# nv-nguyen/gigapose

Hardware: NVIDIA H100
Metric: detections/sec (224x224 crops, 162-template bank) (higher is better)
Workload: dtype f32 (a1, a4, a6: bf16 hi/lo split x3 on tensor cores with fp32 accumulate = fp32-faithful; a5, a7-a9: fp32)

## Files before the change

gigapose_b200/csrc/api.cu:

```cuda
#include "../../include/gigapose_b200.h"
#include "gigapose_kernels.h"

#include <atomic>
#include <dlfcn.h>
#include <cstdarg>
#include <cstdio>
#include <cstdlib>
#include <cstring>
#include <new>
#include <string>

int gp_internal_make_map_nhwc(CUtensorMap* map, void* ptr, uint64_t C, uint64_t W, uint64_t H, uint64_t N, uint32_t out_w,
                              uint32_t out_h, uint32_t stride);
int gp_internal_make_map_raw(CUtensorMap* map, void* ptr, int rank, const uint64_t* dims, const uint64_t* strides_bytes,
                             const uint32_t* box, const uint32_t* elem_strides);
int gp_internal_make_map_ex(CUtensorMap* map, void* ptr, uint64_t rows, uint64_t cols, uint32_t box_cols, uint32_t box_rows,
                            int swizzle_bytes);
int gp_internal_make_map(CUtensorMap* map, void* ptr, uint64_t rows, uint64_t cols, uint32_t box_rows);

namespace {

thread_local std::string g_last_error;
std::atomic<uint64_t> g_launches{0};

int fail(int code, const char* fmt, ...) {
  char buf[512];
  va_list ap;
  va_start(ap, fmt);
  vsnprintf(buf, sizeof(buf), fmt, ap);
  va_end(ap);
  g_last_error = buf;
  return code;
}

#define GP_CUDA(expr)                                                                                     \
  do {                                                                                                    \
    cudaError_t _e = (expr);                                                                              \
    if (_e != cudaSuccess) return fail(GP_ERR_CUDA, "%s failed: %s", #expr, cudaGetErrorString(_e));     \
  } while (0)

constexpr size_t kAlign = 1024;
inline size_t align_up(size_t x) { return (x + kAlign - 1) / kAlign * kAlign; }

struct Carver {
  uint8_t* base;
  size_t off = 0;
  explicit Carver(void* b) : base(static_cast<uint8_t*>(b)) {}
  template <typename T>
  T* take(size_t count) {
    T* p = base ? reinterpret_cast<T*>(base + off) : nullptr;
    off += align_up(count * sizeof(T));
    return p;
  }
};

typedef CUresult (*EncodeTiledFn)(CUtensorMap*, CUtensorMapDataType, cuuint32_t, void*, const cuuint64_t*,
                                  const cuuint64_t*, const cuuint32_t*, const cuuint32_t*, CUtensorMapInterleave,
                                  CUtensorMapSwizzle, CUtensorMapL2promotion, CUtensorMapFloatOOBfill);

EncodeTiledFn get_encode_fn() {
  static EncodeTiledFn fn = nullptr;
  if (!fn) {
    void* p = nullptr;
    cudaDriverEntryPointQueryResult q;
    if (cudaGetDriverEntryPoint("cuTensorMapEncodeTiled", &p, cudaEnableDefault, &q) == cudaSuccess &&
        q == cudaDriverEntryPointSuccess)
      fn = reinterpret_cast<EncodeTiledFn>(p);
  }
  return fn;
}

}

int gp_internal_fail(int code, const char* fmt, ...) {
  char buf[512];
  va_list ap;
  va_start(ap, fmt);
  vsnprintf(buf, sizeof(buf), fmt, ap);
  va_end(ap);
  g_last_error = buf;
  return code;
}
void gp_internal_count_launches(int n) { g_launches += n; }
namespace gp {
bool pdl_enabled() {
  const char* ev = getenv("GIGAPOSE_PDL");
  return ev ? (ev[0] != '0') : false;
}
}

int gp_internal_make_map_ex(CUtensorMap* map, void* ptr, uint64_t rows, uint64_t cols, uint32_t box_cols, uint32_t box_rows,
                            int swizzle_bytes) {
  EncodeTiledFn enc = get_encode_fn();
  if (!enc) return fail(GP_ERR_UNSUPPORTED, "cuTensorMapEncodeTiled not available from this driver");
  cuuint64_t dims[2] = {cols, rows};
  cuuint64_t strides[1] = {cols * sizeof(uint16_t)};
  cuuint32_t box[2] = {box_cols, box_rows};
  cuuint32_t estr[2] = {1, 1};
  const CUtensorMapSwizzle sw = swizzle_bytes == 128 ? CU_TENSOR_MAP_SWIZZLE_128B : CU_TENSOR_MAP_SWIZZLE_64B;
  CUresult r = enc(map, CU_TENSOR_MAP_DATA_TYPE_BFLOAT16, 2, ptr, dims, strides, box, estr, CU_TENSOR_MAP_INTERLEAVE_NONE, sw,
                   CU_TENSOR_MAP_L2_PROMOTION_L2_128B, CU_TENSOR_MAP_FLOAT_OOB_FILL_NONE);
  if (r != CUDA_SUCCESS) return fail(GP_ERR_CUDA, "cuTensorMapEncodeTiled failed with CUresult %d", (int)r);
  return GP_OK;
}
int gp_internal_make_map_nhwc(CUtensorMap* map, void* ptr, uint64_t C, uint64_t W, uint64_t H, uint64_t N, uint32_t out_w,
                              uint32_t out_h, uint32_t stride) {
  EncodeTiledFn enc = get_encode_fn();
  if (!enc) return fail(GP_ERR_UNSUPPORTED, "cuTensorMapEncodeTiled not available from this driver");
  cuuint64_t dims[4] = {C, W, H, N};
  cuuint64_t strides[3] = {C * sizeof(uint16_t), W * C * sizeof(uint16_t), H * W * C * sizeof(uint16_t)};
  cuuint32_t box[4] = {32, out_w * stride, out_h * stride, 1};
  cuuint32_t estr[4] = {1, stride, stride, 1};
  CUresult r = enc(map, CU_TENSOR_MAP_DATA_TYPE_BFLOAT16, 4, ptr, dims, strides, box, estr, CU_TENSOR_MAP_INTERLEAVE_NONE,
                   CU_TENSOR_MAP_SWIZZLE_64B, CU_TENSOR_MAP_L2_PROMOTION_L2_128B, CU_TENSOR_MAP_FLOAT_OOB_FILL_NONE);
  if (r != CUDA_SUCCESS) return fail(GP_ERR_CUDA, "cuTensorMapEncodeTiled (NHWC) failed with CUresult %d", (int)r);
  return GP_OK;
}
int gp_internal_make_map_raw(CUtensorMap* map, void* ptr, int rank, const uint64_t* dims, const uint64_t* strides_bytes,
                             const uint32_t* box, const uint32_t* elem_strides) {
  EncodeTiledFn enc = get_encode_fn();
  if (!enc) return fail(GP_ERR_UNSUPPORTED, "cuTensorMapEncodeTiled not available from this driver");
  cuuint64_t d[5], st[4];
  cuuint32_t b[5], es[5];
  for (int i = 0; i < rank; ++i) { d[i] = dims[i]; b[i] = box[i]; es[i] = elem_strides[i]; if (i + 1 < rank) st[i] = strides_bytes[i]; }
  CUresult r = enc(map, CU_TENSOR_MAP_DATA_TYPE_BFLOAT16, rank, ptr, d, st, b, es, CU_TENSOR_MAP_INTERLEAVE_NONE,
                   CU_TENSOR_MAP_SWIZZLE_64B, CU_TENSOR_MAP_L2_PROMOTION_L2_128B, CU_TENSOR_MAP_FLOAT_OOB_FILL_NONE);
  if (r != CUDA_SUCCESS) return fail(GP_ERR_CUDA, "cuTensorMapEncodeTiled (raw, rank %d) failed with CUresult %d", rank, (int)r);
  return GP_OK;
}
int gp_internal_make_map(CUtensorMap* map, void* ptr, uint64_t rows, uint64_t cols, uint32_t box_rows) {
  return gp_internal_make_map_ex(map, ptr, rows, cols, 32, box_rows, 64);
}

namespace {

int make_plane_map(CUtensorMap* map, void* ptr, uint64_t images, uint32_t box_rows) {
  return gp_internal_make_map_ex(map, ptr, images * 32ull * GP_NUM_PATCHES, 32, 32, box_rows, 64);
}

struct Bank {
  uint16_t *hi, *lo;
  float* mask16;
  float* ist;
  float *K, *M, *pose;
};

struct Workspace {
  uint16_t *q_hi, *q_lo;
  float* q_mask16;
  float* q_ist;
  int *perm, *q_obj;
  float* sim_avg;
  float* rec_score;
  uint8_t *rec_idx, *rec_valid;
  float* c_score; int* c_id; float* c_pts_score; uint8_t *c_idx, *c_valid;
  int* row_count; int* row_ids; float *hidden1, *hidden2;
  uint16_t *mlp_a_hi, *mlp_a_lo;
  uint16_t *w1_hi, *w1_lo, *w2s_hi, *w2s_lo, *w2i_hi, *w2i_lo;
  float* bias1;
};

void carve_bank(Carver& c, const gp_config_t& cfg, Bank* b) {
  const size_t OT = (size_t)cfg.num_objects * cfg.num_templates;
  const size_t OTg = (size_t)cfg.num_objects * cfg.num_templates_global;
  Bank tmp;
  tmp.hi = c.take<uint16_t>(OT * GP_NUM_PATCHES * GP_AE_DIM);
  tmp.lo = c.take<uint16_t>(OT * GP_NUM_PATCHES * GP_AE_DIM);
  tmp.mask16 = c.take<float>(OT * GP_NUM_PATCHES);
  tmp.ist = c.take<float>((cfg.ist_bank_global ? OTg : OT) * GP_NUM_PATCHES * GP_IST_DIM);
  tmp.K = c.take<float>((size_t)cfg.num_objects * 9);
  tmp.M = c.take<float>(OTg * 9);
  tmp.pose = c.take<float>(OTg * 16);
  if (b) *b = tmp;
}

void carve_workspace(Carver& c, const gp_config_t& cfg, Workspace* w) {
  const size_t Bm = cfg.max_batch, T = cfg.num_templates, k = cfg.top_k;
  Workspace tmp;
  tmp.q_hi = c.take<uint16_t>(Bm * GP_NUM_PATCHES * GP_AE_DIM);
  tmp.q_lo = c.take<uint16_t>(Bm * GP_NUM_PATCHES * GP_AE_DIM);
  tmp.q_mask16 = c.take<float>(Bm * GP_NUM_PATCHES);
  tmp.q_ist = c.take<float>(Bm * GP_NUM_PATCHES * GP_IST_DIM);
  tmp.perm = c.take<int>(Bm);
  tmp.q_obj = c.take<int>(Bm);
  tmp.sim_avg = c.take<float>(Bm * T);
  tmp.rec_score = c.take<float>(Bm * T * GP_NUM_PATCHES);
  tmp.rec_idx = c.take<uint8_t>(Bm * T * GP_NUM_PATCHES);
  tmp.rec_valid = c.take<uint8_t>(Bm * T * GP_NUM_PATCHES);
  tmp.c_score = c.take<float>(Bm * k);
  tmp.c_id = c.take<int>(Bm * k);
  tmp.c_pts_score = c.take<float>(Bm * k * GP_NUM_PATCHES);
  tmp.c_idx = c.take<uint8_t>(Bm * k * GP_NUM_PATCHES);
  tmp.c_valid = c.take<uint8_t>(Bm * k * GP_NUM_PATCHES);
  tmp.row_count = c.take<int>(1);
  tmp.row_ids = c.take<int>(Bm * k * GP_NUM_PATCHES);
  tmp.hidden1 = c.take<float>(Bm * k * GP_NUM_PATCHES * 1024);
  tmp.hidden2 = c.take<float>(Bm * k * GP_NUM_PATCHES * 512);
  tmp.mlp_a_hi = c.take<uint16_t>(Bm * k * GP_NUM_PATCHES * 512);
  tmp.mlp_a_lo = c.take<uint16_t>(Bm * k * GP_NUM_PATCHES * 512);
  tmp.w1_hi = c.take<uint16_t>(1024 * 512);
  tmp.w1_lo = c.take<uint16_t>(1024 * 512);
  tmp.w2s_hi = c.take<uint16_t>(256 * 512);
  tmp.w2s_lo = c.take<uint16_t>(256 * 512);
  tmp.w2i_hi = c.take<uint16_t>(256 * 512);
  tmp.w2i_lo = c.take<uint16_t>(256 * 512);
  tmp.bias1 = c.take<float>(1024);
  if (w) *w = tmp;
}

int validate(const gp_config_t* cfg) {
  if (!cfg) return fail(GP_ERR_INVALID, "null config");
  if (cfg->abi_version != GP_ABI_VERSION) return fail(GP_ERR_INVALID, "ABI version mismatch: %d vs %d", cfg->abi_version, GP_ABI_VERSION);
  if (cfg->num_objects < 1 || cfg->num_templates < 1 || cfg->max_batch < 1)
    return fail(GP_ERR_INVALID, "num_objects, num_templates and max_batch must be >= 1");
  if (cfg->top_k < 1 || cfg->top_k > 32) return fail(GP_ERR_INVALID, "top_k must be in [1,32]");
  if (cfg->num_templates_global < cfg->num_templates) return fail(GP_ERR_INVALID, "num_templates_global < num_templates");
  if (cfg->num_templates_global < cfg->top_k) return fail(GP_ERR_INVALID, "fewer templates than top_k (torch.topk would raise)");
  if (cfg->template_id_stride < 1 || cfg->template_id_offset < 0) return fail(GP_ERR_INVALID, "bad template id stride/offset");
  if (cfg->patch_size < 1) return fail(GP_ERR_INVALID, "patch_size must be >= 1");
  if (cfg->sim_threshold != cfg->sim_threshold) return fail(GP_ERR_INVALID, "sim_threshold is NaN");
  if (cfg->precision != GP_PRECISION_FP32_SPLIT && cfg->precision != GP_PRECISION_BF16)
    return fail(GP_ERR_INVALID, "unknown precision %d", cfg->precision);
  if (cfg->ist_bank_global != 0 && cfg->ist_bank_global != 1) return fail(GP_ERR_INVALID, "ist_bank_global must be 0 or 1");
  if ((size_t)cfg->num_objects * cfg->num_templates * GP_NUM_PATCHES * 32 >= (1ull << 31))
    return fail(GP_ERR_INVALID, "bank has too many rows for 32-bit TMA coordinates");
  return GP_OK;
}

}

struct gp_context {
  gp_config_t cfg;
  int num_sms;
  Bank bank;
  Workspace ws;
  CUtensorMap tm_q_hi, tm_q_lo, tm_t_hi, tm_t_lo;
  int mlp_tc;
  CUtensorMap tm_ma_hi, tm_ma_lo;
  CUtensorMap tm_h1s_hi, tm_h1s_lo, tm_h1i_hi, tm_h1i_lo;
  CUtensorMap tm_w1_hi, tm_w1_lo, tm_w2s_hi, tm_w2s_lo, tm_w2i_hi, tm_w2i_lo;
  gp::IstMlpWeights mlp;
  bool mlp_set;
  int cur_B;
  void* nccl_comm;
  int rank, world;
};

namespace {
typedef int (*NcclAllGatherFn)(const void*, void*, size_t, int, void*, cudaStream_t);
typedef const char* (*NcclErrFn)(int);
NcclAllGatherFn g_allgather = nullptr;
NcclErrFn g_nccl_err = nullptr;
int resolve_nccl() {
  if (g_allgather) return GP_OK;
  void* sym = dlsym(RTLD_DEFAULT, "ncclAllGather");
  void* lib = nullptr;
  if (!sym) {
    lib = dlopen("libnccl.so.2", RTLD_NOW | RTLD_GLOBAL);
    if (lib) sym = dlsym(lib, "ncclAllGather");
  }
  if (!sym) return fail(GP_ERR_UNSUPPORTED, "ncclAllGather not found: load libnccl.so.2 (e.g. import torch) before gp_comm_init");
  g_allgather = reinterpret_cast<NcclAllGatherFn>(sym);
  void* es = dlsym(RTLD_DEFAULT, "ncclGetErrorString");
  if (!es && lib) es = dlsym(lib, "ncclGetErrorString");
  g_nccl_err = reinterpret_cast<NcclErrFn>(es);
  return GP_OK;
}
}

extern "C" {

const char* gp_last_error(void) { return g_last_error.c_str(); }
int gp_abi_version(void) { return GP_ABI_VERSION; }
uint64_t gp_launch_count(void) { return g_launches.load(); }

int gp_query_sizes(const gp_config_t* cfg, size_t* bank_bytes, size_t* workspace_bytes) {
  if (int e = validate(cfg)) return e;
  Carver cb(nullptr), cw(nullptr);
  carve_bank(cb, *cfg, nullptr);
  carve_workspace(cw, *cfg, nullptr);
  if (bank_bytes) *bank_bytes = cb.off;
  if (workspace_bytes) *workspace_bytes = cw.off;
  return GP_OK;
}

int gp_create(const gp_config_t* cfg, void* bank_mem, void* workspace_mem, gp_handle_t* out) {
  if (int e = validate(cfg)) return e;
  if (!bank_mem || !workspace_mem || !out) return fail(GP_ERR_INVALID, "null pointer argument");
  if (((uintptr_t)bank_mem | (uintptr_t)workspace_mem) & (kAlign - 1))
    return fail(GP_ERR_INVALID, "bank and workspace must be %zu-byte aligned", kAlign);
  GP_CUDA(cudaSetDevice(cfg->device));
  cudaDeviceProp prop;
  GP_CUDA(cudaGetDeviceProperties(&prop, cfg->device));
  if (prop.major != 9 || prop.minor != 0)
    return fail(GP_ERR_UNSUPPORTED, "device %d is sm_%d%d; this library contains sm_90a code only", cfg->device,
                prop.major, prop.minor);
  if ((int)prop.sharedMemPerBlockOptin < gp::sim_search_smem_bytes())
    return fail(GP_ERR_UNSUPPORTED, "device offers %zu B of shared memory per block, kernel needs %d",
                prop.sharedMemPerBlockOptin, gp::sim_search_smem_bytes());
  gp_context* h = new (std::nothrow) gp_context();
  if (!h) return fail(GP_ERR_INVALID, "out of host memory");
  h->cfg = *cfg;
  h->num_sms = prop.multiProcessorCount;
  h->mlp_set = false;
  h->cur_B = 0;
  {
    const char* ev = getenv("GIGAPOSE_MLP_SIMT");
    h->mlp_tc = ev ? (ev[0] == '0') : 0;
  }
  h->nccl_comm = nullptr;
  h->rank = 0;
  h->world = 1;
  Carver cb(bank_mem), cw(workspace_mem);
  carve_bank(cb, *cfg, &h->bank);
  carve_workspace(cw, *cfg, &h->ws);
  const uint64_t bank_rows = (uint64_t)cfg->num_objects * cfg->num_templates;
  const uint64_t q_rows = (uint64_t)cfg->max_batch;
  int e;
  if ((e = make_plane_map(&h->tm_t_hi, h->bank.hi, bank_rows, 256)) || (e = make_plane_map(&h->tm_t_lo, h->bank.lo, bank_rows, 256)) ||
      (e = make_plane_map(&h->tm_q_hi, h->ws.q_hi, q_rows, 128)) || (e = make_plane_map(&h->tm_q_lo, h->ws.q_lo, q_rows, 128))) {
    delete h;
    return e;
  }
  {
    const uint64_t rows = (uint64_t)cfg->max_batch * cfg->top_k * GP_NUM_PATCHES;
    uint16_t* h1_hi = reinterpret_cast<uint16_t*>(h->ws.hidden1);
    uint16_t* h1_lo = h1_hi + rows * 1024;
    const uint64_t dims[2] = {512, rows}, strides[1] = {1024 * sizeof(uint16_t)};
    const uint32_t box[2] = {32, 128}, estr[2] = {1, 1};
    int e;
    if ((e = gp_internal_make_map(&h->tm_ma_hi, h->ws.mlp_a_hi, rows, 512, 128)) || (e = gp_internal_make_map(&h->tm_ma_lo, h->ws.mlp_a_lo, rows, 512, 128)) ||
        (e = gp_internal_make_map_raw(&h->tm_h1s_hi, h1_hi, 2, dims, strides, box, estr)) ||
        (e = gp_internal_make_map_raw(&h->tm_h1s_lo, h1_lo, 2, dims, strides, box, estr)) ||
        (e = gp_internal_make_map_raw(&h->tm_h1i_hi, h1_hi + 512, 2, dims, strides, box, estr)) ||
        (e = gp_internal_make_map_raw(&h->tm_h1i_lo, h1_lo + 512, 2, dims, strides, box, estr)) ||
        (e = gp_internal_make_map(&h->tm_w1_hi, h->ws.w1_hi, 1024, 512, 256)) || (e = gp_internal_make_map(&h->tm_w1_lo, h->ws.w1_lo, 1024, 512, 256)) ||
        (e = gp_internal_make_map(&h->tm_w2s_hi, h->ws.w2s_hi, 256, 512, 256)) || (e = gp_internal_make_map(&h->tm_w2s_lo, h->ws.w2s_lo, 256, 512, 256)) ||
        (e = gp_internal_make_map(&h->tm_w2i_hi, h->ws.w2i_hi, 256, 512, 256)) || (e = gp_internal_make_map(&h->tm_w2i_lo, h->ws.w2i_lo, 256, 512, 256))) {
      delete h;
      return e;
    }
  }
  *out = h;
  return GP_OK;
}

int gp_destroy(gp_handle_t h) {
  delete h;
  return GP_OK;
}

namespace {
int split_features(const float* feat, int feat_layout, long long n_imgs, int norm_passes, uint16_t* hi, uint16_t* lo, cudaStream_t s) {
  const long long rows = n_imgs * GP_NUM_PATCHES;
  cudaError_t e;
  if (feat_layout == GP_LAYOUT_CHANNEL_MAJOR)
    e = gp::launch_split_descriptors(feat, rows, GP_AE_DIM, GP_NUM_PATCHES, (long long)GP_NUM_PATCHES * GP_AE_DIM, 1, GP_NUM_PATCHES,
                                     norm_passes, 1, hi, lo, nullptr, s);
  else if (feat_layout == GP_LAYOUT_PATCH_MAJOR)
    e = gp::launch_split_descriptors(feat, rows, GP_AE_DIM, GP_NUM_PATCHES, (long long)GP_NUM_PATCHES * GP_AE_DIM, GP_AE_DIM, 1,
                                     norm_passes, 1, hi, lo, nullptr, s);
  else if (feat_layout == GP_LAYOUT_VIT_TOKENS)
    e = gp::launch_split_descriptors(feat + GP_AE_DIM, rows, GP_AE_DIM, GP_NUM_PATCHES, (long long)(GP_NUM_PATCHES + 1) * GP_AE_DIM,
                                     GP_AE_DIM, 1, norm_passes, 1, hi, lo, nullptr, s);
  else
    return fail(GP_ERR_INVALID, "unknown feature layout %d", feat_layout);
  if (e != cudaSuccess) return fail(GP_ERR_CUDA, "descriptor split failed: %s", cudaGetErrorString(e));
  return GP_OK;
}
}

int gp_normalize_patch_tokens(int b, const float* x_prenorm, float* out, void* stream) {
  if (!x_prenorm || !out || b < 1) return fail(GP_ERR_INVALID, "bad argument");
  GP_CUDA(gp::launch_split_descriptors(x_prenorm + GP_AE_DIM, (long long)b * GP_NUM_PATCHES, GP_AE_DIM, GP_NUM_PATCHES,
                                       (long long)(GP_NUM_PATCHES + 1) * GP_AE_DIM, GP_AE_DIM, 1, 1, 0, nullptr, nullptr, out,
                                       static_cast<cudaStream_t>(stream)));
  g_launches += 1;
  return GP_OK;
}

int gp_bank_write(gp_handle_t h, int obj, int tmpl0, int n, const float* feat, int feat_layout, int norm_passes,
                  const float* mask, int H, int W, const float* ist_feat, void* stream) {
  if (!h) return fail(GP_ERR_INVALID, "null handle");
  const gp_config_t& c = h->cfg;
  if (obj < 0 || obj >= c.num_objects || tmpl0 < 0 || n < 1 || tmpl0 + n > c.num_templates)
    return fail(GP_ERR_INVALID, "template range [%d,%d) of object %d outside the bank (%d x %d)", tmpl0, tmpl0 + n, obj,
                c.num_objects, c.num_templates);
  if (!feat || !mask) return fail(GP_ERR_INVALID, "feat and mask are required");
  if (H < 16 || W < 16) return fail(GP_ERR_INVALID, "mask must be at least 16x16");
  if (norm_passes < 0 || norm_passes > 2) return fail(GP_ERR_INVALID, "norm_passes must be 0, 1 or 2");
  cudaStream_t s = static_cast<cudaStream_t>(stream);
  const size_t slot = (size_t)obj * c.num_templates + tmpl0;
  const size_t plane_off = slot * GP_NUM_PATCHES * GP_AE_DIM;
  if (int e = split_features(feat, feat_layout, n, norm_passes, h->bank.hi + plane_off, h->bank.lo + plane_off, s)) return e;
  GP_CUDA(gp::launch_sample_mask16(mask, n, H, W, h->bank.mask16 + slot * GP_NUM_PATCHES, s));
  g_launches += 2;
  if (ist_feat) {
    if (c.ist_bank_global) return fail(GP_ERR_INVALID, "cfg.ist_bank_global = 1: write IST features with gp_bank_write_ist (global ids)");
    GP_CUDA(gp::launch_transpose_cp(ist_feat, n, GP_IST_DIM, h->bank.ist + slot * GP_NUM_PATCHES * GP_IST_DIM, s));
    g_launches += 1;
  }
  return GP_OK;
}

int gp_bank_write_ist(gp_handle_t h, int obj, int tmpl0, int n, const float* ist_feat, int ist_layout, void* stream) {
  if (!h || !ist_feat) return fail(GP_ERR_INVALID, "null argument");
  const gp_config_t& c = h->cfg;
  const int Ti = c.ist_bank_global ? c.num_templates_global : c.num_templates;
  if (obj < 0 || obj >= c.num_objects || tmpl0 < 0 || n < 1 || tmpl0 + n > Ti)
    return fail(GP_ERR_INVALID, "IST template range [%d,%d) of object %d outside the bank (%d x %d)", tmpl0, tmpl0 + n, obj,
                c.num_objects, Ti);
  cudaStream_t s = static_cast<cudaStream_t>(stream);
  float* dst = h->bank.ist + ((size_t)obj * Ti + tmpl0) * GP_NUM_PATCHES * GP_IST_DIM;
  if (ist_layout == GP_LAYOUT_CHANNEL_MAJOR) {
    GP_CUDA(gp::launch_transpose_cp(ist_feat, n, GP_IST_DIM, dst, s));
    g_launches += 1;
  } else if (ist_layout == GP_LAYOUT_PATCH_MAJOR) {
    GP_CUDA(cudaMemcpyAsync(dst, ist_feat, (size_t)n * GP_NUM_PATCHES * GP_IST_DIM * sizeof(float), cudaMemcpyDeviceToDevice, s));
  } else {
    return fail(GP_ERR_INVALID, "unknown IST feature layout %d", ist_layout);
  }
  return GP_OK;
}

int gp_bank_set_poses(gp_handle_t h, const float* K, const float* M, const float* poses, void* stream) {
  if (!h || !K || !M || !poses) return fail(GP_ERR_INVALID, "null argument");
  const gp_config_t& c = h->cfg;
  cudaStream_t s = static_cast<cudaStream_t>(stream);
  const size_t OTg = (size_t)c.num_objects * c.num_templates_global;
  GP_CUDA(cudaMemcpyAsync(h->bank.K, K, (size_t)c.num_objects * 9 * sizeof(float), cudaMemcpyDeviceToDevice, s));
  GP_CUDA(cudaMemcpyAsync(h->bank.M, M, OTg * 9 * sizeof(float), cudaMemcpyDeviceToDevice, s));
  GP_CUDA(cudaMemcpyAsync(h->bank.pose, poses, OTg * 16 * sizeof(float), cudaMemcpyDeviceToDevice, s));
  return GP_OK;
}

static constexpr float kMlpWeightScale = 64.0f;

int gp_set_ist_weights(gp_handle_t h, const float* const w[12], int use_tanh, void* stream) {
  if (!h || !w) return fail(GP_ERR_INVALID, "null argument");
  for (int i = 0; i < 12; ++i)
    if (!w[i]) return fail(GP_ERR_INVALID, "IST weight pointer %d is null", i);
  gp::IstMlpWeights& m = h->mlp;
  m.s_w1 = w[0]; m.s_b1 = w[1]; m.s_w2 = w[2]; m.s_b2 = w[3]; m.s_w3 = w[4]; m.s_b3 = w[5];
  m.i_w1 = w[6]; m.i_b1 = w[7]; m.i_w2 = w[8]; m.i_b2 = w[9]; m.i_w3 = w[10]; m.i_b3 = w[11];
  m.use_tanh = use_tanh;
  cudaStream_t s = static_cast<cudaStream_t>(stream);
  Workspace& ws = h->ws;
  GP_CUDA(gp::launch_split_planes(w[0], 512, 512, 512, ws.w1_hi, ws.w1_lo, s, true, kMlpWeightScale));
  GP_CUDA(gp::launch_split_planes(w[6], 512, 512, 512, ws.w1_hi + 512 * 512, ws.w1_lo + 512 * 512, s, true, kMlpWeightScale));
  GP_CUDA(gp::launch_split_planes(w[2], 256, 512, 512, ws.w2s_hi, ws.w2s_lo, s, true, kMlpWeightScale));
  GP_CUDA(gp::launch_split_planes(w[8], 256, 512, 512, ws.w2i_hi, ws.w2i_lo, s, true, kMlpWeightScale));
  GP_CUDA(cudaMemcpyAsync(ws.bias1, w[1], 512 * sizeof(float), cudaMemcpyDeviceToDevice, s));
  GP_CUDA(cudaMemcpyAsync(ws.bias1 + 512, w[7], 512 * sizeof(float), cudaMemcpyDeviceToDevice, s));
  g_launches += 4;
  h->mlp_set = true;
  return GP_OK;
}

int gp_set_queries(gp_handle_t h, int B, const float* q_feat, int feat_layout, int norm_passes, const float* q_mask,
                   int H, int W, const int32_t* q_obj, void* stream) {
  if (!h || !q_feat || !q_mask || !q_obj) return fail(GP_ERR_INVALID, "null argument");
  if (B < 1 || B > h->cfg.max_batch) return fail(GP_ERR_INVALID, "batch %d outside [1, max_batch=%d]", B, h->cfg.max_batch);
  if (H < 16 || W < 16) return fail(GP_ERR_INVALID, "mask must be at least 16x16");
  if (norm_passes < 0 || norm_passes > 2) return fail(GP_ERR_INVALID, "norm_passes must be 0, 1 or 2");
  cudaStream_t s = static_cast<cudaStream_t>(stream);
  if (int e = split_features(q_feat, feat_layout, B, norm_passes, h->ws.q_hi, h->ws.q_lo, s)) return e;
  GP_CUDA(gp::launch_sample_mask16(q_mask, B, H, W, h->ws.q_mask16, s));
  GP_CUDA(gp::launch_object_order(q_obj, B, h->cfg.num_objects, h->ws.q_obj, h->ws.perm, s));
  g_launches += 3;
  h->cur_B = B;
  return GP_OK;
}

static int run_sim(gp_context* h, int B, cudaStream_t s, float* debug_tile = nullptr) {
  gp::SimSearchParams p;
  p.num_items = B * h->cfg.num_templates;
  p.B = B;
  p.T = h->cfg.num_templates;
  p.perm = h->ws.perm;
  p.q_obj = h->ws.q_obj;
  p.q_mask = h->ws.q_mask16;
  p.bank_mask = h->bank.mask16;
  p.sim_threshold = h->cfg.sim_threshold;
  p.patch_threshold = h->cfg.patch_threshold;
  p.passes = h->cfg.precision == GP_PRECISION_FP32_SPLIT ? 3 : 1;
  p.sim_avg = h->ws.sim_avg;
  p.rec_score = h->ws.rec_score;
  p.rec_idx = h->ws.rec_idx;
  p.rec_valid = h->ws.rec_valid;
  p.debug_tile = debug_tile;
  GP_CUDA(gp::launch_sim_search(h->tm_q_hi, h->tm_q_lo, h->tm_t_hi, h->tm_t_lo, p, h->num_sms, s));
  g_launches += 1;
  return GP_OK;
}

int gp_sim_candidates(gp_handle_t h, int B, const gp_candidates_t* out, void* stream) {
  if (!h || !out) return fail(GP_ERR_INVALID, "null argument");
  if (B != h->cur_B) return fail(GP_ERR_STATE, "gp_set_queries staged %d queries, search asked for %d", h->cur_B, B);
  cudaStream_t s = static_cast<cudaStream_t>(stream);
  if (int e = run_sim(h, B, s)) return e;
  gp::TopkSelectParams t;
  t.B = B; t.T = h->cfg.num_templates; t.k = h->cfg.top_k;
  t.id_stride = h->cfg.template_id_stride; t.id_offset = h->cfg.template_id_offset;
  t.sim_avg = h->ws.sim_avg; t.rec_score = h->ws.rec_score; t.rec_idx = h->ws.rec_idx; t.rec_valid = h->ws.rec_valid;
  t.cand_score = out->score; t.cand_id = out->id; t.cand_pts_score = out->pts_score; t.cand_idx = out->idx;
  t.cand_valid = out->valid;
  GP_CUDA(gp::launch_topk_select(t, s));
  g_launches += 1;
  return GP_OK;
}

int gp_topk_merge(gp_handle_t h, int B, int G, const gp_candidates_t* g, size_t rank_stride_bytes,
                  const gp_matches_t* out, float* out_rel_scale, float* out_rel_inplane, void* stream) {
  if (!h || !g || !out) return fail(GP_ERR_INVALID, "null argument");
  if (B < 1 || G < 1 || G * h->cfg.top_k > 64) return fail(GP_ERR_INVALID, "B=%d G=%d: need G*k <= 64", B, G);
  gp::TopkMergeParams m;
  m.B = B; m.k = h->cfg.top_k; m.G = G; m.rank_stride_bytes = rank_stride_bytes;
  m.cand_score = g->score; m.cand_id = g->id; m.cand_pts_score = g->pts_score; m.cand_idx = g->idx; m.cand_valid = g->valid;
  m.cand_rel_scale = g->rel_scale; m.cand_rel_inplane = g->rel_inplane;
  m.out_rel_scale = out_rel_scale; m.out_rel_inplane = out_rel_inplane;
  m.id_src = reinterpret_cast<long long*>(out->id_src); m.score_src = out->score_src; m.score_pts = out->score_pts;
  m.tar_pts = reinterpret_cast<long long*>(out->tar_pts); m.src_pts = reinterpret_cast<long long*>(out->src_pts);
  GP_CUDA(gp::launch_topk_merge_expand(m, static_cast<cudaStream_t>(stream)));
  g_launches += 1;
  return GP_OK;
}

int gp_sim_topk(gp_handle_t h, int B, const gp_matches_t* out, void* stream) {
  if (!h || !out) return fail(GP_ERR_INVALID, "null argument");
  gp_candidates_t c;
  c.score = h->ws.c_score; c.id = h->ws.c_id; c.pts_score = h->ws.c_pts_score; c.idx = h->ws.c_idx; c.valid = h->ws.c_valid;
  c.rel_scale = nullptr; c.rel_inplane = nullptr;
  if (int e = gp_sim_candidates(h, B, &c, stream)) return e;
  return gp_topk_merge(h, B, 1, &c, 0, out, nullptr, nullptr, stream);
}

int gp_ist_mlp(gp_handle_t h, int b0, int n, const float* q_ist, int ist_layout, const gp_matches_t* m, float* rel_scale,
               float* rel_inplane, void* stream) {
  if (!h || !q_ist || !m || !rel_scale || !rel_inplane) return fail(GP_ERR_INVALID, "null argument");
  if (!h->mlp_set) return fail(GP_ERR_STATE, "gp_set_ist_weights has not been called");
  if (b0 < 0 || n < 1 || b0 + n > h->cur_B)
    return fail(GP_ERR_STATE, "gp_set_queries staged %d queries, gp_ist_mlp asked for [%d,%d)", h->cur_B, b0, b0 + n);
  cudaStream_t s = static_cast<cudaStream_t>(stream);
  const float* q_pm = q_ist;
  if (ist_layout == GP_LAYOUT_CHANNEL_MAJOR) {
    GP_CUDA(gp::launch_transpose_cp(q_ist, n, GP_IST_DIM, h->ws.q_ist, s));
    q_pm = h->ws.q_ist;
    g_launches += 1;
  } else if (ist_layout != GP_LAYOUT_PATCH_MAJOR) {
    return fail(GP_ERR_INVALID, "unknown IST feature layout %d", ist_layout);
  }
  const gp_config_t& c = h->cfg;
  gp::IstMlpParams p;
  p.B = n; p.k = c.top_k;
  if (c.ist_bank_global) { p.T = c.num_templates_global; p.id_stride = 1; p.id_offset = 0; }
  else { p.T = c.num_templates; p.id_stride = c.template_id_stride; p.id_offset = c.template_id_offset; }
  p.id_src = reinterpret_cast<const long long*>(m->id_src);
  p.src_pts = reinterpret_cast<const long long*>(m->src_pts);
  p.tar_pts = reinterpret_cast<const long long*>(m->tar_pts);
  p.q_obj = h->ws.q_obj + b0; p.q_ist = q_pm; p.bank_ist = h->bank.ist;
  p.rel_scale = rel_scale; p.rel_inplane = rel_inplane;
  p.row_count = h->ws.row_count; p.row_ids = h->ws.row_ids; p.hidden1 = h->ws.hidden1; p.hidden2 = h->ws.hidden2;
  if (!h->mlp_tc) {
    GP_CUDA(gp::launch_ist_mlp(h->mlp, p, s));
    g_launches += 4;
    return GP_OK;
  }
  const int rows = n * c.top_k * GP_NUM_PATCHES;
  const uint64_t max_rows = (uint64_t)c.max_batch * c.top_k * GP_NUM_PATCHES;
  uint16_t* h1_hi = reinterpret_cast<uint16_t*>(h->ws.hidden1);
  uint16_t* h1_lo = h1_hi + max_rows * 1024;
  float* h2s = h->ws.hidden2;
  float* h2i = h->ws.hidden2 + max_rows * 256;
  GP_CUDA(gp::launch_mlp_gather_planes(p, h->ws.mlp_a_hi, h->ws.mlp_a_lo, s));
  gp::GemmParams g{};
  g.passes = 3; g.f16 = 1; g.acc_scale = 1.0f / kMlpWeightScale; g.m_dev = h->ws.row_count;
  g.M = rows; g.N = 1024; g.K = 512; g.mode = gp::GEMM_PLANES_RELU; g.bias = h->ws.bias1; g.out_hi = h1_hi; g.out_lo = h1_lo;
  GP_CUDA(gp::launch_vit_gemm(h->tm_ma_hi, h->tm_ma_lo, h->tm_w1_hi, h->tm_w1_lo, g, h->num_sms, s));
  g = gp::GemmParams{};
  g.passes = 3; g.f16 = 1; g.acc_scale = 1.0f / kMlpWeightScale; g.m_dev = h->ws.row_count;
  g.M = rows; g.N = 256; g.K = 512; g.mode = gp::GEMM_ROWS_F32_RELU; g.bias = h->mlp.s_b2; g.x = h2s;
  GP_CUDA(gp::launch_vit_gemm(h->tm_h1s_hi, h->tm_h1s_lo, h->tm_w2s_hi, h->tm_w2s_lo, g, h->num_sms, s));
  g.bias = h->mlp.i_b2; g.x = h2i;
  GP_CUDA(gp::launch_vit_gemm(h->tm_h1i_hi, h->tm_h1i_lo, h->tm_w2i_hi, h->tm_w2i_lo, g, h->num_sms, s));
  GP_CUDA(gp::launch_mlp_head_rows(h->mlp, p, h2s, h2i, s));
  g_launches += 6;
  return GP_OK;
}

int gp_ransac(int n, float pixel_threshold, int patch_size, const int64_t* src_pts, const int64_t* tar_pts,
              const float* rel_scale, const float* rel_inplane, const gp_ransac_out_t* out, void* stream) {
  if (!src_pts || !tar_pts || !rel_scale || !rel_inplane || !out || !out->inlier_count || !out->M || !out->failed ||
      !out->inlier_src_pts || !out->inlier_tar_pts || !out->inlier_scores)
    return fail(GP_ERR_INVALID, "null argument");
  if (n < 1) return fail(GP_ERR_INVALID, "n must be >= 1");
  gp::RansacParams p;
  p.n = n; p.pixel_threshold = pixel_threshold; p.patch_size = patch_size;
  p.src_pts = reinterpret_cast<const long long*>(src_pts);
  p.tar_pts = reinterpret_cast<const long long*>(tar_pts);
  p.rel_scale = rel_scale; p.rel_inplane = rel_inplane;
  p.M = out->M; p.failed = out->failed;
  p.in_src = reinterpret_cast<long long*>(out->inlier_src_pts);
  p.in_tar = reinterpret_cast<long long*>(out->inlier_tar_pts);
  p.in_score = reinterpret_cast<long long*>(out->inlier_scores);
  p.in_count = out->inlier_count;
  GP_CUDA(gp::launch_ransac(p, static_cast<cudaStream_t>(stream)));
  g_launches += 1;
  return GP_OK;
}

int gp_pose_recover(int B, int k, int num_templates, const int32_t* q_obj, const float* q_K, const float* q_M,
                    const int64_t* id_src, const float* M, const float* tmpl_K, const float* tmpl_M,
                    const float* tmpl_pose, float* poses, void* stream) {
  if (!q_obj || !q_K || !q_M || !id_src || !M || !tmpl_K || !tmpl_M || !tmpl_pose || !poses)
    return fail(GP_ERR_INVALID, "null argument");
  if (B < 1 || k < 1 || num_templates < 1) return fail(GP_ERR_INVALID, "B, k and num_templates must be >= 1");
  GP_CUDA(gp::launch_pose_only(B * k, k, num_templates, q_obj, q_K, q_M, reinterpret_cast<const long long*>(id_src), M,
                               tmpl_K, tmpl_M, tmpl_pose, poses, static_cast<cudaStream_t>(stream)));
  g_launches += 1;
  return GP_OK;
}

int gp_sort_and_pose(gp_handle_t h, int b0, int n, int sort_by_inliers, const float* q_K, const float* q_M,
                     const gp_matches_t* m, const float* rel_scale, const float* rel_inplane, const gp_ransac_out_t* r,
                     const gp_predictions_t* o, void* stream) {
  if (!h || !q_K || !q_M || !m || !rel_scale || !rel_inplane || !r || !o) return fail(GP_ERR_INVALID, "null argument");
  if (b0 < 0 || n < 1 || b0 + n > h->cur_B)
    return fail(GP_ERR_STATE, "gp_set_queries staged %d queries, gp_sort_and_pose asked for [%d,%d)", h->cur_B, b0, b0 + n);
  gp::PoseParams p;
  p.B = n; p.k = h->cfg.top_k; p.T = h->cfg.num_templates_global;
  p.sort = sort_by_inliers ? 1 : 0;
  p.q_obj = h->ws.q_obj + b0; p.q_K = q_K; p.q_M = q_M;
  p.tmpl_K = h->bank.K; p.tmpl_M = h->bank.M; p.tmpl_pose = h->bank.pose;
  p.in_count = r->inlier_count;
  p.id_src = reinterpret_cast<const long long*>(m->id_src); p.score_src = m->score_src; p.score_pts = m->score_pts;
  p.tar_pts = reinterpret_cast<const long long*>(m->tar_pts); p.src_pts = reinterpret_cast<const long long*>(m->src_pts);
  p.rel_scale = rel_scale; p.rel_inplane = rel_inplane;
  p.M = r->M; p.failed = r->failed;
  p.in_src = reinterpret_cast<const long long*>(r->inlier_src_pts);
  p.in_tar = reinterpret_cast<const long long*>(r->inlier_tar_pts);
  p.in_score = reinterpret_cast<const long long*>(r->inlier_scores);
  p.o_id_src = reinterpret_cast<long long*>(o->matches.id_src); p.o_score_src = o->matches.score_src;
  p.o_score_pts = o->matches.score_pts;
  p.o_tar_pts = reinterpret_cast<long long*>(o->matches.tar_pts); p.o_src_pts = reinterpret_cast<long long*>(o->matches.src_pts);
  p.o_rel_scale = o->rel_scale; p.o_rel_inplane = o->rel_inplane;
  p.o_M = o->ransac.M; p.o_failed = o->ransac.failed;
  p.o_in_src = reinterpret_cast<long long*>(o->ransac.inlier_src_pts);
  p.o_in_tar = reinterpret_cast<long long*>(o->ransac.inlier_tar_pts);
  p.o_in_score = reinterpret_cast<long long*>(o->ransac.inlier_scores);
  p.o_scores = o->scores; p.o_poses = o->poses;
  GP_CUDA(gp::launch_sort_and_pose(p, static_cast<cudaStream_t>(stream)));
  g_launches += 1;
  return GP_OK;
}

int gp_comm_init(gp_handle_t h, void* nccl_comm, int rank, int world) {
  if (!h || !nccl_comm) return fail(GP_ERR_INVALID, "null argument");
  if (world < 1 || rank < 0 || rank >= world) return fail(GP_ERR_INVALID, "rank %d outside [0, world=%d)", rank, world);
  if (world != h->cfg.template_id_stride || rank != h->cfg.template_id_offset)
    return fail(GP_ERR_INVALID, "communicator (rank %d of %d) does not match the shard map of this handle (offset %d, stride %d)",
                rank, world, h->cfg.template_id_offset, h->cfg.template_id_stride);
  if (world * h->cfg.top_k > 64) return fail(GP_ERR_INVALID, "world * top_k = %d exceeds the merge kernel's 64 candidates", world * h->cfg.top_k);
  if (int e = resolve_nccl()) return e;
  h->nccl_comm = nccl_comm;
  h->rank = rank;
  h->world = world;
  return GP_OK;
}

int gp_allgather(gp_handle_t h, const void* send, void* recv, size_t bytes_per_rank, void* stream) {
  if (!h || !send || !recv) return fail(GP_ERR_INVALID, "null argument");
  if (!h->nccl_comm) return fail(GP_ERR_STATE, "gp_comm_init has not been called");
  const int r = g_allgather(send, recv, bytes_per_rank,  0, h->nccl_comm, static_cast<cudaStream_t>(stream));
  if (r != 0) return fail(GP_ERR_CUDA, "ncclAllGather failed: %s", g_nccl_err ? g_nccl_err(r) : "?");
  return GP_OK;
}

int gp_topk_allgather_merge(gp_handle_t h, int B, void* packed, size_t rank_stride_bytes, const gp_candidates_t* slot0,
                            const gp_matches_t* out, void* stream) {
  if (!h || !packed || !slot0 || !out) return fail(GP_ERR_INVALID, "null argument");
  if (!h->nccl_comm) return fail(GP_ERR_STATE, "gp_comm_init has not been called");
  if (B != h->cur_B) return fail(GP_ERR_STATE, "gp_set_queries staged %d queries, merge asked for %d", h->cur_B, B);
  uint8_t* base = static_cast<uint8_t*>(packed);
  if (int e = gp_allgather(h, base + (size_t)h->rank * rank_stride_bytes, base, rank_stride_bytes, stream)) return e;
  return gp_topk_merge(h, B, h->world, slot0, rank_stride_bytes, out, nullptr, nullptr, stream);
}

int gp_debug_sim_tiles(gp_handle_t h, int B, float* tiles, void* stream) {
  if (!h || !tiles) return fail(GP_ERR_INVALID, "null argument");
  if (B != h->cur_B) return fail(GP_ERR_STATE, "gp_set_queries staged %d queries, debug asked for %d", h->cur_B, B);
  return run_sim(h, B, static_cast<cudaStream_t>(stream), tiles);
}

int gp_time_sim_kernel(gp_handle_t h, int B, int iters, float* avg_ms, void* stream) {
  if (!h || !avg_ms || iters < 1) return fail(GP_ERR_INVALID, "bad argument");
  if (B != h->cur_B) return fail(GP_ERR_STATE, "gp_set_queries staged %d queries, timing asked for %d", h->cur_B, B);
  cudaStream_t s = static_cast<cudaStream_t>(stream);
  cudaEvent_t e0, e1;
  GP_CUDA(cudaEventCreate(&e0));
  GP_CUDA(cudaEventCreate(&e1));
  if (int e = run_sim(h, B, s)) return e;
  GP_CUDA(cudaEventRecord(e0, s));
  for (int i = 0; i < iters; ++i)
    if (int e = run_sim(h, B, s)) return e;
  GP_CUDA(cudaEventRecord(e1, s));
  GP_CUDA(cudaEventSynchronize(e1));
  float ms = 0.f;
  GP_CUDA(cudaEventElapsedTime(&ms, e0, e1));
  cudaEventDestroy(e0);
  cudaEventDestroy(e1);
  *avg_ms = ms / iters;
  return GP_OK;
}

}
```

gigapose_b200/csrc/ist_trunk.cu:

```cuda
#include "../../include/gigapose_b200.h"
#include "gigapose_kernels.h"

#include <cuda_bf16.h>
#include <cstdlib>
#include <new>
#include <vector>

extern int gp_internal_fail(int code, const char* fmt, ...);
extern void gp_internal_count_launches(int n);
extern int gp_internal_make_map(CUtensorMap* map, void* ptr, uint64_t rows, uint64_t cols, uint32_t box_rows);
extern int gp_internal_make_map_raw(CUtensorMap* map, void* ptr, int rank, const uint64_t* dims, const uint64_t* strides_bytes,
                                    const uint32_t* box, const uint32_t* elem_strides);
extern int gp_internal_make_map_nhwc(CUtensorMap* map, void* ptr, uint64_t C, uint64_t W, uint64_t H, uint64_t N,
                                     uint32_t out_w, uint32_t out_h, uint32_t stride);

namespace {

constexpr int kIn = 224, kRes = 256, kStemOut = 128, kStemKPad = 224, kFeat = 256;
constexpr int kPadRows = kRes + 6, kPadCols = kRes + 8;
constexpr int kDims[4] = {128, 192, 256, 512};
constexpr int kNumConvs = GP_IST_TRUNK_NUM_CONVS;
constexpr size_t kAlign = 1024;
inline size_t up(size_t x) { return (x + kAlign - 1) / kAlign * kAlign; }

struct Carver {
  uint8_t* base; size_t off = 0;
  explicit Carver(void* b) : base(static_cast<uint8_t*>(b)) {}
  template <typename T> T* take(size_t n) { T* p = base ? reinterpret_cast<T*>(base + off) : nullptr; off += up(n * sizeof(T)); return p; }
};

struct Planes { uint16_t *hi = nullptr, *lo = nullptr; };

struct Conv {
  int cin, cout, k, stride, pad, hin, hout;
  int K, Kpad, bn, mode;
  int swap;
  int in_buf, out_buf, res_buf;
  Planes w;
  const float* bias;
  CUtensorMap a_hi, a_lo, w_hi, w_lo;
};

std::vector<Conv> make_schedule() {
  std::vector<Conv> v;
  auto add = [&](int cin, int cout, int k, int stride, int pad, int hin, int mode, int in_buf, int out_buf, int res_buf) {
    Conv c{};
    c.cin = cin; c.cout = cout; c.k = k; c.stride = stride; c.pad = pad; c.hin = hin; c.hout = hin / stride;
    c.K = k * k * cin; c.Kpad = cin == 3 ? kStemKPad : c.K;
    c.swap = cout == 128 ? 1 : 0;
    c.bn = cout == 192 ? 192 : 256;
    c.mode = mode; c.in_buf = in_buf; c.out_buf = out_buf; c.res_buf = res_buf;
    v.push_back(c);
  };
  add(3, kStemOut, 7, 2, 3, kRes, gp::GEMM_PLANES_RELU, -1, 0, -1);
  int x = 0, width = kStemOut, h = kStemOut;
  for (int st = 0; st < 4; ++st) {
    const int d = kDims[st];
    for (int blk = 0; blk < 2; ++blk) {
      const int stride = (blk == 0 && st > 0) ? 2 : 1;
      int free_buf[3], nf = 0;
      for (int b = 0; b < 4; ++b) if (b != x) free_buf[nf++] = b;
      const int y = free_buf[0];
      const bool ds = stride != 1;
      const int res = ds ? free_buf[1] : x, z = ds ? free_buf[2] : free_buf[1];
      add(width, d, 3, stride, 1, h, gp::GEMM_PLANES_RELU, x, y, -1);
      if (ds) add(width, d, 1, stride, 0, h, gp::GEMM_PLANES, x, res, -1);
      add(d, d, 3, 1, 1, h / stride, gp::GEMM_PLANES_ADD_RELU, y, z, res);
      x = z; width = d; h /= stride;
    }
  }
  add(kDims[3], kFeat, 1, 1, 0, h, gp::GEMM_ROWS_F32, x, -1, -1);
  return v;
}

#define GPI_CUDA(expr)                                                                                    \
  do {                                                                                                    \
    cudaError_t _e = (expr);                                                                              \
    if (_e != cudaSuccess) return gp_internal_fail(GP_ERR_CUDA, "%s failed: %s", #expr, cudaGetErrorString(_e)); \
  } while (0)

__device__ __forceinline__ void split_store(float v, __nv_bfloat16* hi, __nv_bfloat16* lo, size_t i) {
  const __nv_bfloat16 h = __float2bfloat16_rn(v);
  hi[i] = h;
  lo[i] = __float2bfloat16_rn(v - __bfloat162float(h));
}

__global__ void resize_pad_kernel(const float* __restrict__ img, int n, uint2* __restrict__ hi, uint2* __restrict__ lo) {
  const int i = blockIdx.x * blockDim.x + threadIdx.x;
  if (i >= n * kRes * kRes) return;
  const int im = i / (kRes * kRes), pix = i - im * kRes * kRes, y = pix / kRes, x = pix - y * kRes;
  const float scale = (float)(kIn - 1) / (float)(kRes - 1);
  const float fy = scale * y, fx = scale * x;
  const int y0 = (int)fy, x0 = (int)fx;
  const int yp = y0 < kIn - 1 ? 1 : 0, xp = x0 < kIn - 1 ? 1 : 0;
  const float ly = fy - y0, lx = fx - x0, hy = 1.f - ly, hx = 1.f - lx;
  uint32_t h[3], l[3];
#pragma unroll
  for (int c = 0; c < 3; ++c) {
    const float* src = img + ((size_t)im * 3 + c) * kIn * kIn;
    const float v = hy * (hx * src[y0 * kIn + x0] + lx * src[y0 * kIn + x0 + xp]) +
                    ly * (hx * src[(y0 + yp) * kIn + x0] + lx * src[(y0 + yp) * kIn + x0 + xp]);
    const __nv_bfloat16 b = __float2bfloat16_rn(v);
    h[c] = __bfloat16_as_ushort(b);
    l[c] = __bfloat16_as_ushort(__float2bfloat16_rn(v - __bfloat162float(b)));
  }
  const size_t o = ((size_t)im * kPadRows + y + 3) * kPadCols + x + 4;
  hi[o] = make_uint2(h[0] | (h[1] << 16), h[2]);
  lo[o] = make_uint2(l[0] | (l[1] << 16), l[2]);
}

__global__ void pack_stem_filter_kernel(const float* __restrict__ w, __nv_bfloat16* __restrict__ hi, __nv_bfloat16* __restrict__ lo) {
  const int i = blockIdx.x * blockDim.x + threadIdx.x;
  if (i >= kStemOut * kStemKPad) return;
  const int co = i / kStemKPad, k = i - co * kStemKPad, ky = k >> 5, px = (k >> 2) & 7, c = k & 3;
  split_store(px >= 1 && c < 3 ? w[((co * 7 + ky) * 7 + (px - 1)) * 3 + c] : 0.f, hi, lo, (size_t)i);
}

__global__ void merge_planes_kernel(const __nv_bfloat16* __restrict__ hi, const __nv_bfloat16* __restrict__ lo, long long n,
                                    float* __restrict__ out) {
  const long long i = (long long)blockIdx.x * blockDim.x + threadIdx.x;
  if (i < n) out[i] = __bfloat162float(hi[i]) + __bfloat162float(lo[i]);
}

}

struct gp_ist_trunk_context {
  int max_crops, passes, num_sms;
  std::vector<Conv> convs;
  Planes act[4];
  Planes stem;
  const float* zero_bias;
};

namespace {

void carve_weights(Carver& c, gp_ist_trunk_context* h, const std::vector<Conv>& sched) {
  for (size_t i = 0; i < sched.size(); ++i) {
    const size_t n = (size_t)sched[i].cout * sched[i].Kpad;
    uint16_t* a = c.take<uint16_t>(n); uint16_t* b = c.take<uint16_t>(n);
    if (h) { h->convs[i].w.hi = a; h->convs[i].w.lo = b; }
  }
  const float* z = c.take<float>(512);
  if (h) h->zero_bias = z;
}

void carve_workspace(Carver& c, int max_crops, gp_ist_trunk_context* h) {
  const size_t act = (size_t)max_crops * kStemOut * kStemOut * kDims[0];
  for (int b = 0; b < 4; ++b) {
    uint16_t* a = c.take<uint16_t>(act); uint16_t* l = c.take<uint16_t>(act);
    if (h) { h->act[b].hi = a; h->act[b].lo = l; }
  }
  const size_t st = (size_t)max_crops * kPadRows * kPadCols * 4;
  uint16_t* a = c.take<uint16_t>(st); uint16_t* l = c.take<uint16_t>(st);
  if (h) { h->stem.hi = a; h->stem.lo = l; }
}

int run(gp_ist_trunk_context* h, int n, const float* crops, float* feat, int stop_after, float* dump, cudaStream_t s) {
  resize_pad_kernel<<<(n * kRes * kRes + 255) / 256, 256, 0, s>>>(crops, n, reinterpret_cast<uint2*>(h->stem.hi),
                                                                  reinterpret_cast<uint2*>(h->stem.lo));
  GPI_CUDA(cudaGetLastError());
  int launched = 1;
  const int last = stop_after > 0 && stop_after < (int)h->convs.size() ? stop_after : (int)h->convs.size();
  for (int i = 0; i < last; ++i) {
    const Conv& c = h->convs[i];
    gp::GemmParams g{};
    g.passes = h->passes; g.mode = c.mode; g.bn = c.bn;
    g.M = n * c.hout * c.hout; g.N = c.cout; g.K = c.Kpad;
    if (c.swap) { g.swap = 1; g.M = c.cout; g.N = n * c.hout * c.hout; }
    g.bias = c.bias ? c.bias : h->zero_bias;
    if (c.out_buf >= 0) { g.out_hi = h->act[c.out_buf].hi; g.out_lo = h->act[c.out_buf].lo; }
    else g.x = feat;
    if (c.res_buf >= 0) { g.res_hi = h->act[c.res_buf].hi; g.res_lo = h->act[c.res_buf].lo; }
    if (c.in_buf < 0) {
      g.conv = 1; g.Ho = c.hout; g.Wo = c.hout; g.stride = 2; g.pad = 0; g.kw = 1; g.cblocks = 1;
    } else if (!(c.k == 1 && c.stride == 1)) {
      g.conv = 1; g.Ho = c.hout; g.Wo = c.hout; g.stride = c.stride; g.pad = c.pad; g.kw = c.k; g.cblocks = c.cin / 32;
    }
    if (c.swap) GPI_CUDA(gp::launch_vit_gemm(c.w_hi, c.w_lo, c.a_hi, c.a_lo, g, h->num_sms, s));
    else GPI_CUDA(gp::launch_vit_gemm(c.a_hi, c.a_lo, c.w_hi, c.w_lo, g, h->num_sms, s));
    ++launched;
  }
  if (dump) {
    const Conv& c = h->convs[last - 1];
    if (c.out_buf < 0) return gp_internal_fail(GP_ERR_INVALID, "the last convolution writes `feat` directly; nothing to dump");
    const long long cnt = (long long)n * c.hout * c.hout * c.cout;
    merge_planes_kernel<<<(unsigned)((cnt + 255) / 256), 256, 0, s>>>(
        reinterpret_cast<const __nv_bfloat16*>(h->act[c.out_buf].hi), reinterpret_cast<const __nv_bfloat16*>(h->act[c.out_buf].lo),
        cnt, dump);
    GPI_CUDA(cudaGetLastError());
    ++launched;
  }
  gp_internal_count_launches(launched);
  return GP_OK;
}

}

extern "C" {

int gp_ist_trunk_query_sizes(int max_crops, size_t* weight_bytes, size_t* workspace_bytes) {
  if (max_crops < 1) return gp_internal_fail(GP_ERR_INVALID, "bad max_crops");
  Carver cw(nullptr), cs(nullptr);
  carve_weights(cw, nullptr, make_schedule());
  carve_workspace(cs, max_crops, nullptr);
  if (weight_bytes) *weight_bytes = cw.off;
  if (workspace_bytes) *workspace_bytes = cs.off;
  return GP_OK;
}

int gp_ist_trunk_create(int device, int max_crops, int precision, const gp_conv_weights_t* w, void* weight_mem,
                        void* workspace_mem, void* stream, gp_ist_trunk_handle_t* out) {
  if (max_crops < 1 || !w || !weight_mem || !workspace_mem || !out) return gp_internal_fail(GP_ERR_INVALID, "bad argument");
  if (precision != GP_PRECISION_FP32_SPLIT && precision != GP_PRECISION_BF16)
    return gp_internal_fail(GP_ERR_INVALID, "unknown precision %d", precision);
  if (((uintptr_t)weight_mem | (uintptr_t)workspace_mem) & (kAlign - 1))
    return gp_internal_fail(GP_ERR_INVALID, "weight and workspace memory must be 1024-byte aligned");
  for (int i = 0; i < kNumConvs; ++i)
    if (!w[i].weight) return gp_internal_fail(GP_ERR_INVALID, "weight pointer %d is null", i);
  GPI_CUDA(cudaSetDevice(device));
  cudaDeviceProp prop;
  GPI_CUDA(cudaGetDeviceProperties(&prop, device));
  if (prop.major != 9 || prop.minor != 0) return gp_internal_fail(GP_ERR_UNSUPPORTED, "device %d is not sm_90", device);
  gp_ist_trunk_context* h = new (std::nothrow) gp_ist_trunk_context();
  if (!h) return gp_internal_fail(GP_ERR_INVALID, "out of host memory");
  h->max_crops = max_crops; h->num_sms = prop.multiProcessorCount;
  h->passes = precision == GP_PRECISION_FP32_SPLIT ? 3 : 1;
  h->convs = make_schedule();
  Carver cw(weight_mem), cs(workspace_mem);
  carve_weights(cw, h, h->convs);
  carve_workspace(cs, max_crops, h);
  cudaStream_t s = static_cast<cudaStream_t>(stream);
  cudaError_t ce = cudaMemsetAsync(const_cast<float*>(h->zero_bias), 0, 512 * sizeof(float), s);
  const size_t stem_bytes = (size_t)max_crops * kPadRows * kPadCols * 4 * sizeof(uint16_t);
  if (ce == cudaSuccess) ce = cudaMemsetAsync(h->stem.hi, 0, stem_bytes, s);
  if (ce == cudaSuccess) ce = cudaMemsetAsync(h->stem.lo, 0, stem_bytes, s);
  int e = GP_OK;
  for (int i = 0; i < kNumConvs && !e && ce == cudaSuccess; ++i) {
    Conv& c = h->convs[i];
    c.bias = w[i].bias;
    if (c.in_buf < 0) {
      pack_stem_filter_kernel<<<(kStemOut * kStemKPad + 255) / 256, 256, 0, s>>>(
          w[i].weight, reinterpret_cast<__nv_bfloat16*>(c.w.hi), reinterpret_cast<__nv_bfloat16*>(c.w.lo));
      ce = cudaGetLastError();
    } else {
      ce = gp::launch_split_planes(w[i].weight, c.cout, c.K, c.Kpad, c.w.hi, c.w.lo, s);
    }
    if (ce != cudaSuccess) break;
    const uint32_t wbox = c.swap ? 128 : c.bn, pix_tile = c.swap ? 256 : 128;
    if ((e = gp_internal_make_map(&c.w_hi, c.w.hi, c.cout, c.Kpad, wbox)) || (e = gp_internal_make_map(&c.w_lo, c.w.lo, c.cout, c.Kpad, wbox)))
      break;
    if (c.in_buf < 0) {
      const uint64_t dims[4] = {32, (uint64_t)kStemOut, (uint64_t)kPadRows, (uint64_t)max_crops};
      const uint64_t strides[3] = {16, (uint64_t)kPadCols * 8, (uint64_t)kPadRows * kPadCols * 8};
      const uint32_t box[4] = {32, (uint32_t)kStemOut, (pix_tile / kStemOut) * 2, 1}, es[4] = {1, 1, 2, 1};
      (e = gp_internal_make_map_raw(&c.a_hi, h->stem.hi, 4, dims, strides, box, es)) ||
          (e = gp_internal_make_map_raw(&c.a_lo, h->stem.lo, 4, dims, strides, box, es));
    } else if (c.k == 1 && c.stride == 1) {
      const uint64_t rows = (uint64_t)max_crops * c.hin * c.hin;
      (e = gp_internal_make_map(&c.a_hi, h->act[c.in_buf].hi, rows, c.cin, pix_tile)) ||
          (e = gp_internal_make_map(&c.a_lo, h->act[c.in_buf].lo, rows, c.cin, pix_tile));
    } else {
      const uint32_t ow = c.hout, oh = pix_tile / c.hout;
      (e = gp_internal_make_map_nhwc(&c.a_hi, h->act[c.in_buf].hi, c.cin, c.hin, c.hin, max_crops, ow, oh, c.stride)) ||
          (e = gp_internal_make_map_nhwc(&c.a_lo, h->act[c.in_buf].lo, c.cin, c.hin, c.hin, max_crops, ow, oh, c.stride));
    }
  }
  if (ce != cudaSuccess) { delete h; return gp_internal_fail(GP_ERR_CUDA, "weight packing failed: %s", cudaGetErrorString(ce)); }
  if (e) { delete h; return e; }
  gp_internal_count_launches(kNumConvs);
  *out = h;
  return GP_OK;
}

int gp_ist_trunk_destroy(gp_ist_trunk_handle_t h) {
  delete h;
  return GP_OK;
}

int gp_ist_trunk_forward(gp_ist_trunk_handle_t h, int n, const float* crops, float* feat, void* stream) {
  if (!h || !crops || !feat) return gp_internal_fail(GP_ERR_INVALID, "null argument");
  if (n < 1 || n > h->max_crops) return gp_internal_fail(GP_ERR_INVALID, "batch %d outside [1, %d]", n, h->max_crops);
  return run(h, n, crops, feat, 0, nullptr, static_cast<cudaStream_t>(stream));
}

int gp_debug_ist_trunk(gp_ist_trunk_handle_t h, int n, const float* crops, int num_convs, float* activation, void* stream) {
  if (!h || !crops || !activation) return gp_internal_fail(GP_ERR_INVALID, "null argument");
  if (n < 1 || n > h->max_crops) return gp_internal_fail(GP_ERR_INVALID, "batch %d outside [1, %d]", n, h->max_crops);
  if (num_convs < 1 || num_convs >= kNumConvs) return gp_internal_fail(GP_ERR_INVALID, "num_convs outside [1, %d)", kNumConvs);
  return run(h, n, crops, nullptr, num_convs, activation, static_cast<cudaStream_t>(stream));
}

}
```

gigapose_b200/csrc/vit_api.cu:

```cuda
#include "../../include/gigapose_b200.h"
#include "gigapose_kernels.h"

#include <cstdarg>
#include <cstdio>
#include <cstdlib>
#include <new>
#include <string>
#include <vector>

extern int gp_internal_fail(int code, const char* fmt, ...);
extern void gp_internal_count_launches(int n);
extern int gp_internal_make_map(CUtensorMap* map, void* ptr, uint64_t rows, uint64_t cols, uint32_t box_rows);
extern int gp_internal_make_map_ex(CUtensorMap* map, void* ptr, uint64_t rows, uint64_t cols, uint32_t box_cols,
                                   uint32_t box_rows, int swizzle_bytes);

namespace {

constexpr int kDim = 1024, kQkv = 3072, kMlp = 4096, kTok = 257, kPatchK = 588, kPatchKPad = 608;
constexpr size_t kAlign = 1024;
inline size_t up(size_t x) { return (x + kAlign - 1) / kAlign * kAlign; }

struct Carver {
  uint8_t* base; size_t off = 0;
  explicit Carver(void* b) : base(static_cast<uint8_t*>(b)) {}
  template <typename T> T* take(size_t n) { T* p = base ? reinterpret_cast<T*>(base + off) : nullptr; off += up(n * sizeof(T)); return p; }
};

struct Planes { uint16_t *hi, *lo; CUtensorMap m_hi, m_lo; };

struct BlockW {
  Planes qkv, proj, fc1, fc2;
  const float *n1w, *n1b, *qkv_b, *proj_b, *ls1, *n2w, *n2b, *fc1_b, *fc2_b, *ls2;
};

#define GPV_CUDA(expr)                                                                                    \
  do {                                                                                                    \
    cudaError_t _e = (expr);                                                                              \
    if (_e != cudaSuccess) return gp_internal_fail(GP_ERR_CUDA, "%s failed: %s", #expr, cudaGetErrorString(_e)); \
  } while (0)

}

struct gp_vit_context {
  int depth, max_crops, passes, num_sms;
  Planes patch_w;
  const float *patch_b, *cls, *pos;
  std::vector<BlockW> blocks;
  float* x;
  Planes ln, qkv, attn, hid, patches;
  CUtensorMap qkv_hi128, qkv_lo128, qkv_hi16, qkv_lo16;
  size_t workspace_bytes;
};

namespace {

void carve_weights(Carver& c, int depth, gp_vit_context* h) {
  auto planes = [&](Planes* p, size_t n) { uint16_t* a = c.take<uint16_t>(n); uint16_t* b = c.take<uint16_t>(n); if (p) { p->hi = a; p->lo = b; } };
  planes(h ? &h->patch_w : nullptr, (size_t)kDim * kPatchKPad);
  for (int i = 0; i < depth; ++i) {
    BlockW* b = h ? &h->blocks[i] : nullptr;
    planes(b ? &b->qkv : nullptr, (size_t)kQkv * kDim);
    planes(b ? &b->proj : nullptr, (size_t)kDim * kDim);
    planes(b ? &b->fc1 : nullptr, (size_t)kMlp * kDim);
    planes(b ? &b->fc2 : nullptr, (size_t)kDim * kMlp);
  }
}

void carve_workspace(Carver& c, int max_crops, gp_vit_context* h) {
  const size_t M = (size_t)max_crops * kTok;
  auto planes = [&](Planes* p, size_t n) { uint16_t* a = c.take<uint16_t>(n); uint16_t* b = c.take<uint16_t>(n); if (p) { p->hi = a; p->lo = b; } };
  float* x = c.take<float>(M * kDim);
  if (h) h->x = x;
  planes(h ? &h->ln : nullptr, M * kDim);
  planes(h ? &h->qkv : nullptr, M * kQkv);
  planes(h ? &h->attn : nullptr, M * kDim);
  planes(h ? &h->hid : nullptr, M * kMlp);
  planes(h ? &h->patches : nullptr, (size_t)max_crops * 256 * kPatchKPad);
}

int make_maps(Planes* p, uint64_t rows, uint64_t cols, uint32_t box_rows) {
  if (int e = gp_internal_make_map(&p->m_hi, p->hi, rows, cols, box_rows)) return e;
  return gp_internal_make_map(&p->m_lo, p->lo, rows, cols, box_rows);
}

}

extern "C" {

int gp_vit_query_sizes(int depth, int max_crops, size_t* weight_bytes, size_t* workspace_bytes) {
  if (depth < 1 || depth > 64 || max_crops < 1) return gp_internal_fail(GP_ERR_INVALID, "bad depth / max_crops");
  Carver cw(nullptr), cs(nullptr);
  carve_weights(cw, depth, nullptr);
  carve_workspace(cs, max_crops, nullptr);
  if (weight_bytes) *weight_bytes = cw.off;
  if (workspace_bytes) *workspace_bytes = cs.off;
  return GP_OK;
}

int gp_vit_create(int device, int depth, int max_crops, int precision, const float* const* w, void* weight_mem,
                  void* workspace_mem, void* stream, gp_vit_handle_t* out) {
  if (depth < 1 || depth > 64 || max_crops < 1 || !w || !weight_mem || !workspace_mem || !out)
    return gp_internal_fail(GP_ERR_INVALID, "bad argument");
  if (precision != GP_PRECISION_FP32_SPLIT && precision != GP_PRECISION_BF16)
    return gp_internal_fail(GP_ERR_INVALID, "unknown precision %d", precision);
  if (((uintptr_t)weight_mem | (uintptr_t)workspace_mem) & (kAlign - 1))
    return gp_internal_fail(GP_ERR_INVALID, "weight and workspace memory must be 1024-byte aligned");
  for (int i = 0; i < 4 + 14 * depth; ++i)
    if (!w[i]) return gp_internal_fail(GP_ERR_INVALID, "weight pointer %d is null", i);
  GPV_CUDA(cudaSetDevice(device));
  cudaDeviceProp prop;
  GPV_CUDA(cudaGetDeviceProperties(&prop, device));
  if (prop.major != 9 || prop.minor != 0) return gp_internal_fail(GP_ERR_UNSUPPORTED, "device %d is not sm_90", device);
  gp_vit_context* h = new (std::nothrow) gp_vit_context();
  if (!h) return gp_internal_fail(GP_ERR_INVALID, "out of host memory");
  h->depth = depth; h->max_crops = max_crops; h->num_sms = prop.multiProcessorCount;
  h->passes = precision == GP_PRECISION_FP32_SPLIT ? 3 : 1;
  h->blocks.resize(depth);
  Carver cw(weight_mem), cs(workspace_mem);
  carve_weights(cw, depth, h);
  carve_workspace(cs, max_crops, h);
  cudaStream_t s = static_cast<cudaStream_t>(stream);
  if (cudaMemsetAsync(workspace_mem, 0, cs.off, s) != cudaSuccess) { delete h; return gp_internal_fail(GP_ERR_CUDA, "workspace memset failed"); }

  h->patch_b = w[1]; h->cls = w[2]; h->pos = w[3];
  cudaError_t ce = gp::launch_split_planes(w[0], kDim, kPatchK, kPatchKPad, h->patch_w.hi, h->patch_w.lo, s);
  int e = ce == cudaSuccess ? make_maps(&h->patch_w, kDim, kPatchKPad, 256) : GP_ERR_CUDA;
  for (int i = 0; i < depth && !e && ce == cudaSuccess; ++i) {
    const float* const* b = w + 4 + 14 * i;
    BlockW& B = h->blocks[i];
    B.n1w = b[0]; B.n1b = b[1]; B.qkv_b = b[3]; B.proj_b = b[5]; B.ls1 = b[6];
    B.n2w = b[7]; B.n2b = b[8]; B.fc1_b = b[10]; B.fc2_b = b[12]; B.ls2 = b[13];
    if ((ce = gp::launch_split_planes(b[2], kQkv, kDim, kDim, B.qkv.hi, B.qkv.lo, s)) != cudaSuccess) break;
    if ((ce = gp::launch_split_planes(b[4], kDim, kDim, kDim, B.proj.hi, B.proj.lo, s)) != cudaSuccess) break;
    if ((ce = gp::launch_split_planes(b[9], kMlp, kDim, kDim, B.fc1.hi, B.fc1.lo, s)) != cudaSuccess) break;
    if ((ce = gp::launch_split_planes(b[11], kDim, kMlp, kMlp, B.fc2.hi, B.fc2.lo, s)) != cudaSuccess) break;
    if ((e = make_maps(&B.qkv, kQkv, kDim, 256)) || (e = make_maps(&B.proj, kDim, kDim, 256)) ||
        (e = make_maps(&B.fc1, kMlp, kDim, 256)) || (e = make_maps(&B.fc2, kDim, kMlp, 256)))
      break;
  }
  const uint64_t M = (uint64_t)max_crops * kTok;
  if (!e && ce == cudaSuccess)
    (e = make_maps(&h->ln, M, kDim, 128)) || (e = make_maps(&h->attn, M, kDim, 128)) || (e = make_maps(&h->hid, M, kMlp, 128)) ||
        (e = make_maps(&h->patches, (uint64_t)max_crops * 256, kPatchKPad, 128)) ||
        (e = gp_internal_make_map_ex(&h->qkv_hi128, h->qkv.hi, 48 * M, 64, 64, 128, 128)) ||
        (e = gp_internal_make_map_ex(&h->qkv_lo128, h->qkv.lo, 48 * M, 64, 64, 128, 128)) ||
        (e = gp_internal_make_map_ex(&h->qkv_hi16, h->qkv.hi, 48 * M, 64, 64, 16, 128)) ||
        (e = gp_internal_make_map_ex(&h->qkv_lo16, h->qkv.lo, 48 * M, 64, 64, 16, 128));
  if (ce != cudaSuccess) { delete h; return gp_internal_fail(GP_ERR_CUDA, "weight packing failed: %s", cudaGetErrorString(ce)); }
  if (e) { delete h; return e; }
  gp_internal_count_launches(1 + 4 * depth);
  *out = h;
  return GP_OK;
}

int gp_debug_attention_timeline(long long* stamps32) {
  if (!stamps32) return gp_internal_fail(GP_ERR_INVALID, "null argument");
  GPV_CUDA(cudaDeviceSynchronize());
  GPV_CUDA(gp::read_attention_stamps(stamps32));
  return GP_OK;
}

int gp_debug_gemm_timeline(long long* stamps64) {
  if (!stamps64) return gp_internal_fail(GP_ERR_INVALID, "null argument");
  GPV_CUDA(cudaDeviceSynchronize());
  GPV_CUDA(gp::read_gemm_stamps(stamps64));
  return GP_OK;
}

int gp_debug_gemm(const gp_debug_gemm_t* d, void* stream) {
  if (!d) return gp_internal_fail(GP_ERR_INVALID, "null argument");
  gp::GemmParams g{};
  g.M = d->M; g.N = d->N; g.K = d->K; g.bn = d->bn; g.passes = d->passes; g.mode = d->mode; g.swap = d->swap; g.f16 = d->f16;
  g.acc_scale = d->acc_scale; g.bias = d->bias; g.gamma = d->gamma; g.x = d->x; g.out_hi = d->out_hi; g.out_lo = d->out_lo;
  g.pos = d->pos; g.res_hi = d->res_hi; g.res_lo = d->res_lo; g.m_dev = d->m_dev;
  g.tokens_per_img = d->tokens_per_img; g.patches_per_img = d->patches_per_img; g.qkv_crop_stride = d->qkv_crop_stride;
  if (g.M < 1) return gp_internal_fail(GP_ERR_INVALID, "M must be >= 1");
  const char* why = nullptr;
  if (!gp::gemm_config_supported(g, &why)) return gp_internal_fail(GP_ERR_INVALID, "unsupported GEMM: %s", why);
  if (!d->a_hi || !d->a_lo || !d->w_hi || !d->w_lo || !d->bias) return gp_internal_fail(GP_ERR_INVALID, "null operand or bias");
  const bool planes_out = g.mode == gp::GEMM_PLANES || g.mode == gp::GEMM_PLANES_GELU || g.mode == gp::GEMM_QKV_HEADS ||
                          g.mode == gp::GEMM_PLANES_RELU || g.mode == gp::GEMM_PLANES_ADD_RELU;
  if (planes_out ? (!g.out_hi || !g.out_lo) : !g.x) return gp_internal_fail(GP_ERR_INVALID, "null output");
  if (g.mode == gp::GEMM_SCALE_RESIDUAL && !g.gamma) return gp_internal_fail(GP_ERR_INVALID, "null gamma");
  if (g.mode == gp::GEMM_PLANES_ADD_RELU && (!g.res_hi || !g.res_lo)) return gp_internal_fail(GP_ERR_INVALID, "null residual planes");
  if (g.mode == gp::GEMM_PATCH_EMBED && (!g.pos || g.patches_per_img < 1 || g.tokens_per_img <= g.patches_per_img))
    return gp_internal_fail(GP_ERR_INVALID, "patch embedding needs pos and tokens_per_img > patches_per_img >= 1");
  if (g.mode == gp::GEMM_QKV_HEADS && (g.N != kQkv || g.tokens_per_img < 1 || g.qkv_crop_stride * g.tokens_per_img < g.M))
    return gp_internal_fail(GP_ERR_INVALID, "QKV scatter needs N = 3072 and qkv_crop_stride * tokens_per_img >= M");
  if (g.swap && g.m_dev) return gp_internal_fail(GP_ERR_INVALID, "m_dev is not supported with swap");
  int dev = 0, sms = 0;
  GPV_CUDA(cudaGetDevice(&dev));
  GPV_CUDA(cudaDeviceGetAttribute(&sms, cudaDevAttrMultiProcessorCount, dev));
  const int bn = g.bn > 0 ? g.bn : 256;
  CUtensorMap a_hi, a_lo, w_hi, w_lo;
  auto* a_h = const_cast<uint16_t*>(d->a_hi); auto* a_l = const_cast<uint16_t*>(d->a_lo);
  auto* w_h = const_cast<uint16_t*>(d->w_hi); auto* w_l = const_cast<uint16_t*>(d->w_lo);
  if (int e = gp_internal_make_map(&a_hi, a_h, g.M, g.K, 128)) return e;
  if (int e = gp_internal_make_map(&a_lo, a_l, g.M, g.K, 128)) return e;
  if (int e = gp_internal_make_map(&w_hi, w_h, g.N, g.K, bn)) return e;
  if (int e = gp_internal_make_map(&w_lo, w_l, g.N, g.K, bn)) return e;
  GPV_CUDA(gp::launch_vit_gemm(a_hi, a_lo, w_hi, w_lo, g, sms, static_cast<cudaStream_t>(stream)));
  gp_internal_count_launches(1);
  return GP_OK;
}

int gp_debug_attention(int b, int crop_stride, int passes, const uint16_t* qkv_hi, const uint16_t* qkv_lo, uint16_t* out_hi,
                       uint16_t* out_lo, void* stream) {
  if (!qkv_hi || !qkv_lo || !out_hi || !out_lo) return gp_internal_fail(GP_ERR_INVALID, "null argument");
  if (b < 1 || crop_stride < b) return gp_internal_fail(GP_ERR_INVALID, "need 1 <= b (%d) <= crop_stride (%d)", b, crop_stride);
  if (passes != 1 && passes != 3) return gp_internal_fail(GP_ERR_INVALID, "passes must be 1 or 3");
  const uint64_t rows = 48ull * crop_stride * kTok;
  auto* qh = const_cast<uint16_t*>(qkv_hi); auto* ql = const_cast<uint16_t*>(qkv_lo);
  CUtensorMap hi128, lo128, hi16, lo16;
  if (int e = gp_internal_make_map_ex(&hi128, qh, rows, 64, 64, 128, 128)) return e;
  if (int e = gp_internal_make_map_ex(&lo128, ql, rows, 64, 64, 128, 128)) return e;
  if (int e = gp_internal_make_map_ex(&hi16, qh, rows, 64, 64, 16, 128)) return e;
  if (int e = gp_internal_make_map_ex(&lo16, ql, rows, 64, 64, 16, 128)) return e;
  GPV_CUDA(gp::launch_attention_tc(hi128, lo128, hi16, lo16, qkv_hi, qkv_lo, out_hi, out_lo, b, crop_stride, passes,
                                   static_cast<cudaStream_t>(stream)));
  gp_internal_count_launches(1);
  return GP_OK;
}

int gp_vit_destroy(gp_vit_handle_t h) {
  delete h;
  return GP_OK;
}

int gp_vit_time_linears(gp_vit_handle_t h, int b, int iters, float* avg_ms, void* stream) {
  if (!h || !avg_ms || iters < 1) return gp_internal_fail(GP_ERR_INVALID, "bad argument");
  if (b < 1 || b > h->max_crops) return gp_internal_fail(GP_ERR_INVALID, "batch %d outside [1, %d]", b, h->max_crops);
  cudaStream_t s = static_cast<cudaStream_t>(stream);
  const int M = b * kTok;
  auto linear = [&](const Planes& a, const Planes& w, gp::GemmParams& gp_) {
    return gp::launch_vit_gemm(a.m_hi, a.m_lo, w.m_hi, w.m_lo, gp_, h->num_sms, s);
  };
  auto run = [&]() -> int {
    for (int i = 0; i < h->depth; ++i) {
      const BlockW& B = h->blocks[i];
      gp::GemmParams g{};
      g.passes = h->passes; g.M = M; g.N = kQkv; g.K = kDim; g.mode = gp::GEMM_QKV_HEADS; g.bias = B.qkv_b;
      g.out_hi = h->qkv.hi; g.out_lo = h->qkv.lo; g.tokens_per_img = kTok; g.qkv_crop_stride = h->max_crops;
      GPV_CUDA(linear(h->ln, B.qkv, g));
      g = gp::GemmParams{}; g.passes = h->passes;
      g.M = M; g.N = kDim; g.K = kDim; g.mode = gp::GEMM_SCALE_RESIDUAL; g.bias = B.proj_b; g.gamma = B.ls1; g.x = h->x;
      GPV_CUDA(linear(h->attn, B.proj, g));
      g = gp::GemmParams{}; g.passes = h->passes;
      g.M = M; g.N = kMlp; g.K = kDim; g.mode = gp::GEMM_PLANES_GELU; g.bias = B.fc1_b; g.out_hi = h->hid.hi; g.out_lo = h->hid.lo;
      GPV_CUDA(linear(h->ln, B.fc1, g));
      g = gp::GemmParams{}; g.passes = h->passes;
      g.M = M; g.N = kDim; g.K = kMlp; g.mode = gp::GEMM_SCALE_RESIDUAL; g.bias = B.fc2_b; g.gamma = B.ls2; g.x = h->x;
      GPV_CUDA(linear(h->hid, B.fc2, g));
    }
    return GP_OK;
  };
  cudaEvent_t e0, e1;
  GPV_CUDA(cudaEventCreate(&e0));
  GPV_CUDA(cudaEventCreate(&e1));
  if (int e = run()) return e;
  GPV_CUDA(cudaEventRecord(e0, s));
  for (int it = 0; it < iters; ++it)
    if (int e = run()) return e;
  GPV_CUDA(cudaEventRecord(e1, s));
  GPV_CUDA(cudaEventSynchronize(e1));
  float ms = 0.f;
  GPV_CUDA(cudaEventElapsedTime(&ms, e0, e1));
  cudaEventDestroy(e0);
  cudaEventDestroy(e1);
  *avg_ms = ms / iters;
  gp_internal_count_launches(4 * h->depth * (iters + 1));
  return GP_OK;
}

int gp_vit_forward(gp_vit_handle_t h, int b, const float* img, float* x_prenorm, void* stream) {
  if (!h || !img || !x_prenorm) return gp_internal_fail(GP_ERR_INVALID, "null argument");
  if (b < 1 || b > h->max_crops) return gp_internal_fail(GP_ERR_INVALID, "batch %d outside [1, %d]", b, h->max_crops);
  cudaStream_t s = static_cast<cudaStream_t>(stream);
  const int M = b * kTok;
  GPV_CUDA(gp::launch_im2col(img, b, kPatchKPad, h->patches.hi, h->patches.lo, s));
  gp::GemmParams g{};
  g.passes = h->passes; g.tokens_per_img = kTok; g.patches_per_img = 256;
  g.M = b * 256; g.N = kDim; g.K = kPatchKPad; g.mode = gp::GEMM_PATCH_EMBED; g.bias = h->patch_b; g.pos = h->pos; g.x = h->x;
  GPV_CUDA(gp::launch_vit_gemm(h->patches.m_hi, h->patches.m_lo, h->patch_w.m_hi, h->patch_w.m_lo, g, h->num_sms, s));
  GPV_CUDA(gp::launch_cls_rows(h->cls, h->pos, b, h->x, s));
  auto linear = [&](const Planes& a, const Planes& w, gp::GemmParams& gp_) {
    return gp::launch_vit_gemm(a.m_hi, a.m_lo, w.m_hi, w.m_lo, gp_, h->num_sms, s);
  };
  for (int i = 0; i < h->depth; ++i) {
    const BlockW& B = h->blocks[i];
    GPV_CUDA(gp::launch_layernorm_planes(h->x, M, B.n1w, B.n1b, 1e-6f, h->ln.hi, h->ln.lo, s));
    g = gp::GemmParams{}; g.passes = h->passes;
    g.M = M; g.N = kQkv; g.K = kDim; g.mode = gp::GEMM_QKV_HEADS; g.bias = B.qkv_b; g.out_hi = h->qkv.hi; g.out_lo = h->qkv.lo;
    g.tokens_per_img = kTok; g.qkv_crop_stride = h->max_crops;
    GPV_CUDA(linear(h->ln, B.qkv, g));
    GPV_CUDA(gp::launch_attention_tc(h->qkv_hi128, h->qkv_lo128, h->qkv_hi16, h->qkv_lo16, h->qkv.hi, h->qkv.lo,
                                     h->attn.hi, h->attn.lo, b, h->max_crops, h->passes, s));
    g = gp::GemmParams{}; g.passes = h->passes;
    g.M = M; g.N = kDim; g.K = kDim; g.mode = gp::GEMM_SCALE_RESIDUAL; g.bias = B.proj_b; g.gamma = B.ls1; g.x = h->x;
    GPV_CUDA(linear(h->attn, B.proj, g));
    GPV_CUDA(gp::launch_layernorm_planes(h->x, M, B.n2w, B.n2b, 1e-6f, h->ln.hi, h->ln.lo, s));
    g = gp::GemmParams{}; g.passes = h->passes;
    g.M = M; g.N = kMlp; g.K = kDim; g.mode = gp::GEMM_PLANES_GELU; g.bias = B.fc1_b; g.out_hi = h->hid.hi; g.out_lo = h->hid.lo;
    GPV_CUDA(linear(h->ln, B.fc1, g));
    g = gp::GemmParams{}; g.passes = h->passes;
    g.M = M; g.N = kDim; g.K = kMlp; g.mode = gp::GEMM_SCALE_RESIDUAL; g.bias = B.fc2_b; g.gamma = B.ls2; g.x = h->x;
    GPV_CUDA(linear(h->hid, B.fc2, g));
  }
  GPV_CUDA(cudaMemcpyAsync(x_prenorm, h->x, (size_t)M * kDim * sizeof(float), cudaMemcpyDeviceToDevice, s));
  gp_internal_count_launches(3 + 7 * h->depth);
  return GP_OK;
}

}
```

gigapose_b200/csrc/vit_gemm.cu:

```cuda
#include "gigapose_kernels.h"
#include "common.cuh"
#include "wgmma.cuh"
#include <cuda_bf16.h>
#include <cuda_fp16.h>

namespace gp {

namespace {

constexpr int kBlockK = 32;
constexpr int kRowBytes = kBlockK * 2;
constexpr int kStages = 4;
constexpr int kBM = 128, kBN = 256;
constexpr int kAPlane = kBM * kRowBytes;
constexpr int kWPlane = kBN * kRowBytes;
constexpr int kStageBytes = 2 * kAPlane + 2 * kWPlane;
constexpr int kEpiWarps = 8;
constexpr int kThreads = 4 * 32 + kEpiWarps * 32;
constexpr int kAccPitch = kBN + 4;
static_assert(kBM * kAccPitch * 4 <= kStages * kStageBytes, "the staged accumulator lives in the operand ring");

struct __align__(8) GemmSmemTail {
  float bias_s[2][kBN];
  float gamma_s[2][kBN];
  uint8_t stage_buf[kEpiWarps][32 * 80];
  uint64_t full_bar[kStages];
  uint64_t empty_bar[kStages];
  uint64_t ring_free_bar;
};
constexpr int kSmemBytes = 1024 + kStages * kStageBytes + sizeof(GemmSmemTail);

constexpr int kGroupM = 16;
__device__ __forceinline__ void tile_coords(int tile, int num_m, int num_n, int& m_tile, int& n_tile) {
  const int per_group = kGroupM * num_n;
  const int g = tile / per_group, idx = tile - g * per_group;
  const int m_first = g * kGroupM;
  const int gm = min(kGroupM, num_m - m_first);
  n_tile = idx / gm;
  m_tile = m_first + (idx - n_tile * gm);
}

__device__ __forceinline__ float gelu_erf(float x) {
  const float ax = fabsf(x);
  float t, e;
  asm("rcp.approx.ftz.f32 %0, %1;" : "=f"(t) : "f"(fmaf(0.231641888f, ax, 1.0f)));
  asm("ex2.approx.ftz.f32 %0, %1;" : "=f"(e) : "f"(x * x * -0.72134752f));
  float poly = fmaf(1.061405429f, t, -1.453152027f);
  poly = fmaf(poly, t, 1.421413741f);
  poly = fmaf(poly, t, -0.284496736f);
  poly = fmaf(poly, t, 0.254829592f);
  const float q = poly * t * e;
  return 0.5f * x * (x < 0.f ? q : 2.0f - q);
}

__device__ __forceinline__ uint32_t pack_bf16(__nv_bfloat16 a, __nv_bfloat16 b) {
  return (uint32_t)__bfloat16_as_ushort(a) | ((uint32_t)__bfloat16_as_ushort(b) << 16);
}

}

__device__ long long g_gemm_stamp[64];
#define GSTAMP(i) do { if (blockIdx.x == 0 && p.N == 3072 && (i) < 64) g_gemm_stamp[i] = clock64(); } while (0)

template <int kN, bool kF16>
__device__ __forceinline__ void gemm_kblock(float (&d)[kN / 2], uint32_t a_hi, uint32_t a_lo, uint32_t w_hi, uint32_t w_lo,
                                            int passes, bool first) {
#pragma unroll
  for (int pass = 0; pass < 3; ++pass) {
    if (pass < passes) {
      const uint32_t a = (pass == 2 ? a_lo : a_hi), w = (pass == 1 ? w_lo : w_hi);
#pragma unroll
      for (int k16 = 0; k16 < kBlockK / 16; ++k16) {
        const uint64_t da = wgmma_desc_kmajor<kRowBytes>(a + k16 * 32), dw = wgmma_desc_kmajor<kRowBytes>(w + k16 * 32);
        const uint32_t accum = (!first || pass != 0 || k16 != 0) ? 1u : 0u;
        if constexpr (kN == 256) { if constexpr (kF16) wgmma_ss_n256_f16(d, da, dw, accum); else wgmma_ss_n256_bf16(d, da, dw, accum); }
        if constexpr (kN == 192) { if constexpr (kF16) wgmma_ss_n192_f16(d, da, dw, accum); else wgmma_ss_n192_bf16(d, da, dw, accum); }
      }
    }
  }
}

template <bool kSwap, int kTileN, bool kF16, int kMode>
__global__ void __launch_bounds__(kThreads, 1)
vit_gemm_kernel(const __grid_constant__ CUtensorMap tm_a_hi, const __grid_constant__ CUtensorMap tm_a_lo,
                const __grid_constant__ CUtensorMap tm_w_hi, const __grid_constant__ CUtensorMap tm_w_lo, GemmParams p) {
  extern __shared__ uint8_t smem_raw[];
  pdl_trigger();
  uint8_t* smem = smem_raw + ((1024u - (smem_u32(smem_raw) & 1023u)) & 1023u);
  GemmSmemTail& tail = *reinterpret_cast<GemmSmemTail*>(smem + kStages * kStageBytes);
  float* acc_s = reinterpret_cast<float*>(smem);
  const int warp = threadIdx.x >> 5, lane = threadIdx.x & 31;
  const int passes = p.passes;
  constexpr int bn = kTileN;
  const int M_rows = p.m_dev ? min(*p.m_dev, p.M) : p.M;
  const int num_m = (M_rows + kBM - 1) / kBM, num_n = p.N / bn;
  const int num_tiles = num_m * num_n;
  const int num_kb = p.K / kBlockK;

  if (threadIdx.x == 0) {
    for (int s = 0; s < kStages; ++s) { mbar_init(&tail.full_bar[s], 1); mbar_init(&tail.empty_bar[s], kEpiWarps); }
    mbar_init(&tail.ring_free_bar, kEpiWarps);
    fence_barrier_init();
  }
  if (warp == 0 && lane == 0) {
    tma_prefetch_desc(&tm_a_hi); tma_prefetch_desc(&tm_w_hi);
    if (passes == 3) { tma_prefetch_desc(&tm_a_lo); tma_prefetch_desc(&tm_w_lo); }
  }
  __syncthreads();
  pdl_wait();
  if (threadIdx.x == 0) GSTAMP(63);

  if (warp == 0) {
    if (lane == 0) {
      int stage = 0; uint32_t phase = 0, unit = 0;
      const uint32_t tx = (passes == 3 ? 2 : 1) * (kAPlane + bn * kRowBytes);
      for (int tile = blockIdx.x; tile < num_tiles; tile += gridDim.x, ++unit) {
        int mt, nt;
        tile_coords(tile, num_m, num_n, mt, nt);
        const int m0 = mt * kBM, n0 = nt * bn;
        int img = 0, y0 = 0;
        if (p.conv) { const int hw = p.Ho * p.Wo, pix0 = kSwap ? n0 : m0; img = pix0 / hw; y0 = (pix0 - img * hw) / p.Wo; }
        if (unit > 0) mbar_wait(&tail.ring_free_bar, (unit - 1) & 1u);
        for (int kb = 0; kb < num_kb; ++kb) {
          mbar_wait(&tail.empty_bar[stage], phase ^ 1);
          uint8_t* st = smem + stage * kStageBytes;
          mbar_arrive_expect_tx(&tail.full_bar[stage], tx);
          int cb = 0, cx = 0, cy = 0;
          if (p.conv) {
            const int tap = kb / p.cblocks;
            cb = kb - tap * p.cblocks;
            const int ky = tap / p.kw, kx = tap - ky * p.kw;
            cx = kx - p.pad; cy = y0 * p.stride + ky - p.pad;
          }
          auto load2 = [&](void* dst, const CUtensorMap* map, int c0, int c1) { tma_load_2d(dst, map, &tail.full_bar[stage], c0, c1); };
          auto load4 = [&](void* dst, const CUtensorMap* map) {
            tma_load_4d(dst, map, &tail.full_bar[stage], cb * kBlockK, cx, cy, img);
          };
          if (p.conv && !kSwap) {
            load4(st, &tm_a_hi);
            if (passes == 3) load4(st + kAPlane, &tm_a_lo);
          } else {
            load2(st, &tm_a_hi, kb * kBlockK, m0);
            if (passes == 3) load2(st + kAPlane, &tm_a_lo, kb * kBlockK, m0);
          }
          if (p.conv && kSwap) {
            load4(st + 2 * kAPlane, &tm_w_hi);
            if (passes == 3) load4(st + 2 * kAPlane + kWPlane, &tm_w_lo);
          } else {
            load2(st + 2 * kAPlane, &tm_w_hi, kb * kBlockK, n0);
            if (passes == 3) load2(st + 2 * kAPlane + kWPlane, &tm_w_lo, kb * kBlockK, n0);
          }
          if (++stage == kStages) { stage = 0; phase ^= 1; }
        }
      }
    }
  } else if (warp >= 4) {
    const int e = warp - 4, q = e & 3, ch = e >> 2;
    const int r = q * 32 + lane;
    const int etid = e * 32 + lane;
    const int wg = e >> 2, wl = e & 3;
    int stage = 0; uint32_t phase = 0, unit = 0;
    for (int tile = blockIdx.x; tile < num_tiles; tile += gridDim.x, ++unit) {
      const uint32_t acc_i = unit & 1u;
      int mt, nt;
      tile_coords(tile, num_m, num_n, mt, nt);
      if (e == 0 && lane == 0) GSTAMP(unit * 4 + 0);
      float frag[kTileN / 2];
      int prev_stage = -1;
      for (int kb = 0; kb < num_kb; ++kb) {
        mbar_wait(&tail.full_bar[stage], phase);
        const uint32_t st = smem_u32(smem + stage * kStageBytes);
        const uint32_t a_hi = st + wg * (kAPlane / 2), a_lo = a_hi + kAPlane;
        const uint32_t w_hi = st + 2 * kAPlane, w_lo = w_hi + kWPlane;
        acc_fence(frag);
        wgmma_fence();
        gemm_kblock<kTileN, kF16>(frag, a_hi, a_lo, w_hi, w_lo, passes, kb == 0);
        wgmma_commit();
        wgmma_wait<1>();
        if (prev_stage >= 0 && lane == 0) mbar_arrive(&tail.empty_bar[prev_stage]);
        prev_stage = stage;
        if (++stage == kStages) { stage = 0; phase ^= 1; }
      }
      wgmma_wait<0>();
      acc_fence(frag);
      if (lane == 0) mbar_arrive(&tail.empty_bar[prev_stage]);
      if (e == 0 && lane == 0) GSTAMP(unit * 4 + 1);
      named_barrier_sync(1, kEpiWarps * 32);
      {
        const int row0 = wg * 64 + wl * 16 + (lane >> 2), col0 = 2 * (lane & 3);
#pragma unroll
        for (int j8 = 0; j8 < kTileN / 8; ++j8) {
          {
            *reinterpret_cast<float2*>(acc_s + row0 * kAccPitch + j8 * 8 + col0) = make_float2(frag[4 * j8], frag[4 * j8 + 1]);
            *reinterpret_cast<float2*>(acc_s + (row0 + 8) * kAccPitch + j8 * 8 + col0) = make_float2(frag[4 * j8 + 2], frag[4 * j8 + 3]);
          }
        }
      }
      const int ntile0 = nt * bn;
      if (!kSwap && etid < bn) {
        tail.bias_s[acc_i][etid] = __ldg(p.bias + ntile0 + etid);
        if (kMode == GEMM_SCALE_RESIDUAL) tail.gamma_s[acc_i][etid] = __ldg(p.gamma + ntile0 + etid);
      }
      named_barrier_sync(1, kEpiWarps * 32);
      if (e == 0 && lane == 0) GSTAMP(unit * 4 + 2);
      const uint32_t acc = acc_i;
      const int m = mt * kBM + r;
      const int half_cols = bn >> 1;
      const int n0 = ntile0 + ch * half_cols;
      const float* sb = tail.bias_s[acc] + ch * half_cols;
      const float* sg = tail.gamma_s[acc] + ch * half_cols;
      const bool row_ok = m < M_rows;
      size_t out_row = (size_t)m;
      const float* pos_row = nullptr;
      if (kMode == GEMM_PATCH_EMBED) {
        const int img = m / p.patches_per_img, pp = m - img * p.patches_per_img;
        out_row = (size_t)img * p.tokens_per_img + 1 + pp;
        pos_row = p.pos + (size_t)(1 + pp) * p.N;
      }

      uint8_t* stg = tail.stage_buf[e];
      const unsigned okmask = __ballot_sync(0xffffffffu, row_ok);
      auto store_rows_64B = [&](const uint32_t (&w)[16], uint8_t* base, size_t row_byte_off) {
        uint4* srow = reinterpret_cast<uint4*>(stg + lane * 80);
#pragma unroll
        for (int j = 0; j < 4; ++j) srow[j] = make_uint4(w[4 * j], w[4 * j + 1], w[4 * j + 2], w[4 * j + 3]);
        __syncwarp();
        const uint32_t off_lo = (uint32_t)row_byte_off, off_hi = (uint32_t)(row_byte_off >> 32);
#pragma unroll
        for (int it = 0; it < 4; ++it) {
          const int rr = it * 8 + (lane >> 2), piece = lane & 3;
          const uint4 val = *reinterpret_cast<const uint4*>(stg + rr * 80 + piece * 16);
          const size_t o = ((size_t)__shfl_sync(0xffffffffu, off_hi, rr) << 32) | __shfl_sync(0xffffffffu, off_lo, rr);
          if ((okmask >> rr) & 1u) *reinterpret_cast<uint4*>(base + o + piece * 16) = val;
        }
        __syncwarp();
      };
      auto load_rows_64B = [&](uint32_t (&w)[16], const uint8_t* base, size_t row_byte_off) {
        const uint32_t off_lo = (uint32_t)row_byte_off, off_hi = (uint32_t)(row_byte_off >> 32);
#pragma unroll
        for (int it = 0; it < 4; ++it) {
          const int rr = it * 8 + (lane >> 2), piece = lane & 3;
          const size_t o = ((size_t)__shfl_sync(0xffffffffu, off_hi, rr) << 32) | __shfl_sync(0xffffffffu, off_lo, rr);
          uint4 val = make_uint4(0, 0, 0, 0);
          if ((okmask >> rr) & 1u) val = *reinterpret_cast<const uint4*>(base + o + piece * 16);
          *reinterpret_cast<uint4*>(stg + rr * 80 + piece * 16) = val;
        }
        __syncwarp();
        const uint4* srow = reinterpret_cast<const uint4*>(stg + lane * 80);
#pragma unroll
        for (int j = 0; j < 4; ++j) { const uint4 t = srow[j]; w[4 * j] = t.x; w[4 * j + 1] = t.y; w[4 * j + 2] = t.z; w[4 * j + 3] = t.w; }
        __syncwarp();
      };

      auto process_swapped = [&](uint32_t (&v32)[32], int c0) {
        const size_t pix = (size_t)(n0 + c0);
        const size_t cbase = (size_t)(mt * kBM + q * 32);
        const float bias_r = __ldg(p.bias + m);
        float v[32];
#pragma unroll
        for (int j = 0; j < 32; ++j) v[j] = __uint_as_float(v32[j]) + bias_r;
        auto rows_in = [&](const uint16_t* plane) {
#pragma unroll
          for (int it = 0; it < 4; ++it) {
            const int rr = it * 8 + (lane >> 2), piece = lane & 3;
            *reinterpret_cast<uint4*>(stg + rr * 80 + piece * 16) =
                *reinterpret_cast<const uint4*>(reinterpret_cast<const uint8_t*>(plane) + ((pix + rr) * p.M + cbase) * 2 + piece * 16);
          }
          __syncwarp();
#pragma unroll
          for (int j = 0; j < 32; ++j)
            v[j] += __uint_as_float((uint32_t)*reinterpret_cast<const uint16_t*>(stg + j * 80 + lane * 2) << 16);
          __syncwarp();
        };
        if (kMode == GEMM_PLANES_ADD_RELU) { rows_in(p.res_hi); rows_in(p.res_lo); }
        if (kMode == GEMM_PLANES_RELU || kMode == GEMM_PLANES_ADD_RELU) {
#pragma unroll
          for (int j = 0; j < 32; ++j) v[j] = fmaxf(v[j], 0.f);
        }
        auto rows_out = [&](uint16_t* plane, bool low) {
#pragma unroll
          for (int j = 0; j < 32; ++j) {
            const __nv_bfloat16 h = __float2bfloat16_rn(v[j]);
            const __nv_bfloat16 o = low ? __float2bfloat16_rn(v[j] - __bfloat162float(h)) : h;
            *reinterpret_cast<uint16_t*>(stg + j * 80 + lane * 2) = __bfloat16_as_ushort(o);
          }
          __syncwarp();
#pragma unroll
          for (int it = 0; it < 4; ++it) {
            const int rr = it * 8 + (lane >> 2), piece = lane & 3;
            *reinterpret_cast<uint4*>(reinterpret_cast<uint8_t*>(plane) + ((pix + rr) * p.M + cbase) * 2 + piece * 16) =
                *reinterpret_cast<const uint4*>(stg + rr * 80 + piece * 16);
          }
          __syncwarp();
        };
        rows_out(p.out_hi, false);
        rows_out(p.out_lo, true);
      };

      auto process = [&](uint32_t (&v32)[32], int c0) {
        if constexpr (kSwap) { process_swapped(v32, c0); return; }
        const int n = n0 + c0;
        float v[32];
#pragma unroll
        for (int j = 0; j < 32; ++j)
          v[j] = (p.acc_scale != 0.f ? __uint_as_float(v32[j]) * p.acc_scale : __uint_as_float(v32[j])) + sb[c0 + j];
        if (kMode == GEMM_PLANES || kMode == GEMM_PLANES_GELU || kMode == GEMM_QKV_HEADS || kMode == GEMM_PLANES_RELU ||
            kMode == GEMM_PLANES_ADD_RELU) {
          uint32_t hi[16], lo[16];
          if (kMode == GEMM_PLANES_ADD_RELU) {
            const size_t rb = (out_row * p.N + n) * 2;
            load_rows_64B(hi, reinterpret_cast<const uint8_t*>(p.res_hi), rb);
            load_rows_64B(lo, reinterpret_cast<const uint8_t*>(p.res_lo), rb);
#pragma unroll
            for (int j = 0; j < 16; ++j) {
              v[2 * j] += __uint_as_float(hi[j] << 16) + __uint_as_float(lo[j] << 16);
              v[2 * j + 1] += __uint_as_float(hi[j] & 0xffff0000u) + __uint_as_float(lo[j] & 0xffff0000u);
            }
          }
#pragma unroll
          for (int j = 0; j < 32; j += 2) {
            float a = v[j], b = v[j + 1];
            if (kMode == GEMM_PLANES_GELU) { a = gelu_erf(a); b = gelu_erf(b); }
            if (kMode == GEMM_PLANES_RELU || kMode == GEMM_PLANES_ADD_RELU) { a = fmaxf(a, 0.f); b = fmaxf(b, 0.f); }
            if constexpr (kF16) {
              a = fminf(fmaxf(a, -65504.f), 65504.f);
              b = fminf(fmaxf(b, -65504.f), 65504.f);
              const __half ah = __float2half_rn(a), bh = __float2half_rn(b);
              hi[j >> 1] = (uint32_t)__half_as_ushort(ah) | ((uint32_t)__half_as_ushort(bh) << 16);
              lo[j >> 1] = (uint32_t)__half_as_ushort(__float2half_rn(a - __half2float(ah))) |
                           ((uint32_t)__half_as_ushort(__float2half_rn(b - __half2float(bh))) << 16);
            } else {
              const __nv_bfloat16 ah = __float2bfloat16_rn(a), bh = __float2bfloat16_rn(b);
              hi[j >> 1] = pack_bf16(ah, bh);
              lo[j >> 1] = pack_bf16(__float2bfloat16_rn(a - __bfloat162float(ah)), __float2bfloat16_rn(b - __bfloat162float(bh)));
            }
          }
          size_t dst = out_row * p.N + n;
          if (kMode == GEMM_QKV_HEADS) {
            const int which = n >> 10, head = (n & 1023) >> 6, d0 = n & 63;
            const int img = m / p.tokens_per_img, tok = m - img * p.tokens_per_img;
            dst = ((((size_t)which * p.qkv_crop_stride + img) * 16 + head) * p.tokens_per_img + tok) * 64 + d0;
          }
          store_rows_64B(hi, reinterpret_cast<uint8_t*>(p.out_hi), dst * 2);
          store_rows_64B(lo, reinterpret_cast<uint8_t*>(p.out_lo), dst * 2);
        } else if (kMode == GEMM_SCALE_RESIDUAL) {
          const size_t rowb = (out_row * p.N + n) * 4;
#pragma unroll
          for (int half = 0; half < 2; ++half) {
            uint32_t w[16];
            load_rows_64B(w, reinterpret_cast<const uint8_t*>(p.x), rowb + half * 64);
#pragma unroll
            for (int j = 0; j < 16; ++j)
              w[j] = __float_as_uint(__uint_as_float(w[j]) + sg[c0 + half * 16 + j] * v[half * 16 + j]);
            store_rows_64B(w, reinterpret_cast<uint8_t*>(p.x), rowb + half * 64);
          }
        } else if (kMode == GEMM_ROWS_F32 || kMode == GEMM_ROWS_F32_RELU) {
          const size_t rowb = (out_row * p.N + n) * 4;
          const float floor_v = kMode == GEMM_ROWS_F32_RELU ? 0.f : -INFINITY;
#pragma unroll
          for (int half = 0; half < 2; ++half) {
            uint32_t w[16];
#pragma unroll
            for (int j = 0; j < 16; ++j) w[j] = __float_as_uint(fmaxf(v[half * 16 + j], floor_v));
            store_rows_64B(w, reinterpret_cast<uint8_t*>(p.x), rowb + half * 64);
          }
        } else {
          const size_t rowb = (out_row * p.N + n) * 4;
#pragma unroll
          for (int half = 0; half < 2; ++half) {
            uint32_t w[16];
#pragma unroll
            for (int j = 0; j < 16; ++j)
              w[j] = __float_as_uint(v[half * 16 + j] + (row_ok ? __ldg(pos_row + n + half * 16 + j) : 0.f));
            store_rows_64B(w, reinterpret_cast<uint8_t*>(p.x), rowb + half * 64);
          }
        }
      };

      const float* arow = acc_s + r * kAccPitch + ch * half_cols;
      for (int c0 = 0; c0 < half_cols; c0 += 32) {
        uint32_t v[32];
#pragma unroll
        for (int j = 0; j < 8; ++j) {
          const uint4 t = *reinterpret_cast<const uint4*>(arow + c0 + 4 * j);
          v[4 * j] = t.x; v[4 * j + 1] = t.y; v[4 * j + 2] = t.z; v[4 * j + 3] = t.w;
        }
        process(v, c0);
      }
      fence_proxy_async();
      __syncwarp();
      if (lane == 0) mbar_arrive(&tail.ring_free_bar);
      if (e == 0 && lane == 0) GSTAMP(unit * 4 + 3);
    }
  }
}

cudaError_t read_gemm_stamps(long long* host64) { return cudaMemcpyFromSymbol(host64, g_gemm_stamp, sizeof(long long) * 64); }

namespace {
template <bool kSwap, int kTileN, bool kF16, int kMode>
cudaError_t launch_mode(const CUtensorMap& a_hi, const CUtensorMap& a_lo, const CUtensorMap& w_hi, const CUtensorMap& w_lo,
                        const GemmParams& p, int grid, cudaStream_t stream) {
  auto kernel = vit_gemm_kernel<kSwap, kTileN, kF16, kMode>;
  static bool configured = false;
  if (!configured) {
    cudaError_t e = cudaFuncSetAttribute(kernel, cudaFuncAttributeMaxDynamicSharedMemorySize, kSmemBytes);
    if (e != cudaSuccess) return e;
    configured = true;
  }
  return launch_ex(kernel, dim3(grid), dim3(kThreads), kSmemBytes, stream, 1, true, a_hi, a_lo, w_hi, w_lo, p);
}
}

bool gemm_config_supported(const GemmParams& p, const char** why) {
  if (why) *why = nullptr;
  auto no = [&](const char* msg) { if (why) *why = msg; return false; };
  const int bn = p.bn > 0 ? p.bn : kBN;
  const bool plane_mode = p.mode == GEMM_PLANES || p.mode == GEMM_PLANES_RELU || p.mode == GEMM_PLANES_ADD_RELU;
  if (bn != 192 && bn != 256) return no("bn must be 192 or 256 (0 = 256)");
  if (p.N <= 0 || p.N % bn != 0) return no("N must be a positive multiple of bn");
  if (p.K <= 0 || p.K % kBlockK != 0) return no("K must be a positive multiple of 32");
  if (p.passes != 1 && p.passes != 3) return no("passes must be 1 or 3");
  if (p.mode < GEMM_PLANES || p.mode > GEMM_ROWS_F32_RELU) return no("unknown mode");
  const int tile_pixels = p.swap ? bn : kBM;
  if (p.conv && (p.Wo <= 0 || tile_pixels % p.Wo != 0 || p.M % kBM != 0 || p.cblocks <= 0))
    return no("convolution geometry does not tile");
  if (p.swap && (bn != kBN || p.M % kBM != 0 || p.f16 || !plane_mode))
    return no("swap needs bn = 256, M % 128 == 0, bf16 planes and a plane mode without GELU");
  if (p.f16 && (bn != kBN || (p.mode != GEMM_PLANES_RELU && p.mode != GEMM_ROWS_F32_RELU)))
    return no("f16 needs bn = 256 and mode PLANES_RELU or ROWS_F32_RELU");
  if (bn == 192 && !plane_mode) return no("bn = 192 supports the modes PLANES, PLANES_RELU and PLANES_ADD_RELU only");
  return true;
}

cudaError_t launch_vit_gemm(const CUtensorMap& a_hi, const CUtensorMap& a_lo, const CUtensorMap& w_hi,
                            const CUtensorMap& w_lo, const GemmParams& p, int num_sms, cudaStream_t stream) {
  if (p.M <= 0) return cudaSuccess;
  if (!gemm_config_supported(p)) return cudaErrorInvalidValue;
  const int bn = p.bn > 0 ? p.bn : kBN;
  const int tiles = ((p.M + kBM - 1) / kBM) * (p.N / bn);
  const int grid = tiles < num_sms ? tiles : num_sms;
#define GP_GEMM_CASE(SWAP, N, F16, MODE) \
  case MODE: return launch_mode<SWAP, N, F16, MODE>(a_hi, a_lo, w_hi, w_lo, p, grid, stream);
#define GP_GEMM_PLANE_MODES(SWAP, N)            \
  switch (p.mode) {                             \
    GP_GEMM_CASE(SWAP, N, false, GEMM_PLANES)      \
    GP_GEMM_CASE(SWAP, N, false, GEMM_PLANES_RELU) \
    GP_GEMM_CASE(SWAP, N, false, GEMM_PLANES_ADD_RELU) \
    default: return cudaErrorInvalidValue;      \
  }
  if (p.swap) GP_GEMM_PLANE_MODES(true, 256)
  if (p.f16) {
    switch (p.mode) {
      GP_GEMM_CASE(false, 256, true, GEMM_PLANES_RELU)
      GP_GEMM_CASE(false, 256, true, GEMM_ROWS_F32_RELU)
      default: return cudaErrorInvalidValue;
    }
  }
  if (bn == 192) GP_GEMM_PLANE_MODES(false, 192)
  switch (p.mode) {
    GP_GEMM_CASE(false, 256, false, GEMM_PLANES)
    GP_GEMM_CASE(false, 256, false, GEMM_PLANES_GELU)
    GP_GEMM_CASE(false, 256, false, GEMM_SCALE_RESIDUAL)
    GP_GEMM_CASE(false, 256, false, GEMM_PATCH_EMBED)
    GP_GEMM_CASE(false, 256, false, GEMM_QKV_HEADS)
    GP_GEMM_CASE(false, 256, false, GEMM_PLANES_RELU)
    GP_GEMM_CASE(false, 256, false, GEMM_PLANES_ADD_RELU)
    GP_GEMM_CASE(false, 256, false, GEMM_ROWS_F32)
    GP_GEMM_CASE(false, 256, false, GEMM_ROWS_F32_RELU)
    default: return cudaErrorInvalidValue;
  }
#undef GP_GEMM_PLANE_MODES
#undef GP_GEMM_CASE
}

}
```

gigapose_b200/csrc/wgmma.cuh:

```cuda
#pragma once
#include <stdint.h>

namespace gp {

__device__ __forceinline__ void wgmma_ss_n16_bf16(float (&d)[8], uint64_t da, uint64_t db, uint32_t scale_d) {
  asm volatile(
      "{\n\t.reg .pred p;\n\t"
      "setp.ne.b32 p, %10, 0;\n\t"
      "wgmma.mma_async.sync.aligned.m64n16k16.f32.bf16.bf16 "
      "{%0, %1, %2, %3, %4, %5, %6, %7}, "
      "%8, %9, p, 1, 1, 0, 0;\n\t}"
      : "+f"(d[0]), "+f"(d[1]), "+f"(d[2]), "+f"(d[3]), "+f"(d[4]), "+f"(d[5]), "+f"(d[6]), "+f"(d[7])
      : "l"(da), "l"(db), "r"(scale_d));
}
__device__ __forceinline__ void wgmma_ss_n16_f16(float (&d)[8], uint64_t da, uint64_t db, uint32_t scale_d) {
  asm volatile(
      "{\n\t.reg .pred p;\n\t"
      "setp.ne.b32 p, %10, 0;\n\t"
      "wgmma.mma_async.sync.aligned.m64n16k16.f32.f16.f16 "
      "{%0, %1, %2, %3, %4, %5, %6, %7}, "
      "%8, %9, p, 1, 1, 0, 0;\n\t}"
      : "+f"(d[0]), "+f"(d[1]), "+f"(d[2]), "+f"(d[3]), "+f"(d[4]), "+f"(d[5]), "+f"(d[6]), "+f"(d[7])
      : "l"(da), "l"(db), "r"(scale_d));
}
__device__ __forceinline__ void wgmma_ss_n64_bf16(float (&d)[32], uint64_t da, uint64_t db, uint32_t scale_d) {
  asm volatile(
      "{\n\t.reg .pred p;\n\t"
      "setp.ne.b32 p, %34, 0;\n\t"
      "wgmma.mma_async.sync.aligned.m64n64k16.f32.bf16.bf16 "
      "{%0, %1, %2, %3, %4, %5, %6, %7, %8, %9, %10, %11, %12, %13, %14, %15, %16, %17, %18, %19, %20, %21, %22, %23, %24, %25, %26, %27, %28, %29, %30, %31}, "
      "%32, %33, p, 1, 1, 0, 0;\n\t}"
      : "+f"(d[0]), "+f"(d[1]), "+f"(d[2]), "+f"(d[3]), "+f"(d[4]), "+f"(d[5]), "+f"(d[6]), "+f"(d[7]), "+f"(d[8]), "+f"(d[9]), "+f"(d[10]), "+f"(d[11]), "+f"(d[12]), "+f"(d[13]), "+f"(d[14]), "+f"(d[15]), "+f"(d[16]), "+f"(d[17]), "+f"(d[18]), "+f"(d[19]), "+f"(d[20]), "+f"(d[21]), "+f"(d[22]), "+f"(d[23]), "+f"(d[24]), "+f"(d[25]), "+f"(d[26]), "+f"(d[27]), "+f"(d[28]), "+f"(d[29]), "+f"(d[30]), "+f"(d[31])
      : "l"(da), "l"(db), "r"(scale_d));
}
__device__ __forceinline__ void wgmma_ss_n64_f16(float (&d)[32], uint64_t da, uint64_t db, uint32_t scale_d) {
  asm volatile(
      "{\n\t.reg .pred p;\n\t"
      "setp.ne.b32 p, %34, 0;\n\t"
      "wgmma.mma_async.sync.aligned.m64n64k16.f32.f16.f16 "
      "{%0, %1, %2, %3, %4, %5, %6, %7, %8, %9, %10, %11, %12, %13, %14, %15, %16, %17, %18, %19, %20, %21, %22, %23, %24, %25, %26, %27, %28, %29, %30, %31}, "
      "%32, %33, p, 1, 1, 0, 0;\n\t}"
      : "+f"(d[0]), "+f"(d[1]), "+f"(d[2]), "+f"(d[3]), "+f"(d[4]), "+f"(d[5]), "+f"(d[6]), "+f"(d[7]), "+f"(d[8]), "+f"(d[9]), "+f"(d[10]), "+f"(d[11]), "+f"(d[12]), "+f"(d[13]), "+f"(d[14]), "+f"(d[15]), "+f"(d[16]), "+f"(d[17]), "+f"(d[18]), "+f"(d[19]), "+f"(d[20]), "+f"(d[21]), "+f"(d[22]), "+f"(d[23]), "+f"(d[24]), "+f"(d[25]), "+f"(d[26]), "+f"(d[27]), "+f"(d[28]), "+f"(d[29]), "+f"(d[30]), "+f"(d[31])
      : "l"(da), "l"(db), "r"(scale_d));
}
__device__ __forceinline__ void wgmma_ss_n192_bf16(float (&d)[96], uint64_t da, uint64_t db, uint32_t scale_d) {
  asm volatile(
      "{\n\t.reg .pred p;\n\t"
      "setp.ne.b32 p, %98, 0;\n\t"
      "wgmma.mma_async.sync.aligned.m64n192k16.f32.bf16.bf16 "
      "{%0, %1, %2, %3, %4, %5, %6, %7, %8, %9, %10, %11, %12, %13, %14, %15, %16, %17, %18, %19, %20, %21, %22, %23, %24, %25, %26, %27, %28, %29, %30, %31, %32, %33, %34, %35, %36, %37, %38, %39, %40, %41, %42, %43, %44, %45, %46, %47, %48, %49, %50, %51, %52, %53, %54, %55, %56, %57, %58, %59, %60, %61, %62, %63, %64, %65, %66, %67, %68, %69, %70, %71, %72, %73, %74, %75, %76, %77, %78, %79, %80, %81, %82, %83, %84, %85, %86, %87, %88, %89, %90, %91, %92, %93, %94, %95}, "
      "%96, %97, p, 1, 1, 0, 0;\n\t}"
      : "+f"(d[0]), "+f"(d[1]), "+f"(d[2]), "+f"(d[3]), "+f"(d[4]), "+f"(d[5]), "+f"(d[6]), "+f"(d[7]), "+f"(d[8]), "+f"(d[9]), "+f"(d[10]), "+f"(d[11]), "+f"(d[12]), "+f"(d[13]), "+f"(d[14]), "+f"(d[15]), "+f"(d[16]), "+f"(d[17]), "+f"(d[18]), "+f"(d[19]), "+f"(d[20]), "+f"(d[21]), "+f"(d[22]), "+f"(d[23]), "+f"(d[24]), "+f"(d[25]), "+f"(d[26]), "+f"(d[27]), "+f"(d[28]), "+f"(d[29]), "+f"(d[30]), "+f"(d[31]), "+f"(d[32]), "+f"(d[33]), "+f"(d[34]), "+f"(d[35]), "+f"(d[36]), "+f"(d[37]), "+f"(d[38]), "+f"(d[39]), "+f"(d[40]), "+f"(d[41]), "+f"(d[42]), "+f"(d[43]), "+f"(d[44]), "+f"(d[45]), "+f"(d[46]), "+f"(d[47]), "+f"(d[48]), "+f"(d[49]), "+f"(d[50]), "+f"(d[51]), "+f"(d[52]), "+f"(d[53]), "+f"(d[54]), "+f"(d[55]), "+f"(d[56]), "+f"(d[57]), "+f"(d[58]), "+f"(d[59]), "+f"(d[60]), "+f"(d[61]), "+f"(d[62]), "+f"(d[63]), "+f"(d[64]), "+f"(d[65]), "+f"(d[66]), "+f"(d[67]), "+f"(d[68]), "+f"(d[69]), "+f"(d[70]), "+f"(d[71]), "+f"(d[72]), "+f"(d[73]), "+f"(d[74]), "+f"(d[75]), "+f"(d[76]), "+f"(d[77]), "+f"(d[78]), "+f"(d[79]), "+f"(d[80]), "+f"(d[81]), "+f"(d[82]), "+f"(d[83]), "+f"(d[84]), "+f"(d[85]), "+f"(d[86]), "+f"(d[87]), "+f"(d[88]), "+f"(d[89]), "+f"(d[90]), "+f"(d[91]), "+f"(d[92]), "+f"(d[93]), "+f"(d[94]), "+f"(d[95])
      : "l"(da), "l"(db), "r"(scale_d));
}
__device__ __forceinline__ void wgmma_ss_n192_f16(float (&d)[96], uint64_t da, uint64_t db, uint32_t scale_d) {
  asm volatile(
      "{\n\t.reg .pred p;\n\t"
      "setp.ne.b32 p, %98, 0;\n\t"
      "wgmma.mma_async.sync.aligned.m64n192k16.f32.f16.f16 "
      "{%0, %1, %2, %3, %4, %5, %6, %7, %8, %9, %10, %11, %12, %13, %14, %15, %16, %17, %18, %19, %20, %21, %22, %23, %24, %25, %26, %27, %28, %29, %30, %31, %32, %33, %34, %35, %36, %37, %38, %39, %40, %41, %42, %43, %44, %45, %46, %47, %48, %49, %50, %51, %52, %53, %54, %55, %56, %57, %58, %59, %60, %61, %62, %63, %64, %65, %66, %67, %68, %69, %70, %71, %72, %73, %74, %75, %76, %77, %78, %79, %80, %81, %82, %83, %84, %85, %86, %87, %88, %89, %90, %91, %92, %93, %94, %95}, "
      "%96, %97, p, 1, 1, 0, 0;\n\t}"
      : "+f"(d[0]), "+f"(d[1]), "+f"(d[2]), "+f"(d[3]), "+f"(d[4]), "+f"(d[5]), "+f"(d[6]), "+f"(d[7]), "+f"(d[8]), "+f"(d[9]), "+f"(d[10]), "+f"(d[11]), "+f"(d[12]), "+f"(d[13]), "+f"(d[14]), "+f"(d[15]), "+f"(d[16]), "+f"(d[17]), "+f"(d[18]), "+f"(d[19]), "+f"(d[20]), "+f"(d[21]), "+f"(d[22]), "+f"(d[23]), "+f"(d[24]), "+f"(d[25]), "+f"(d[26]), "+f"(d[27]), "+f"(d[28]), "+f"(d[29]), "+f"(d[30]), "+f"(d[31]), "+f"(d[32]), "+f"(d[33]), "+f"(d[34]), "+f"(d[35]), "+f"(d[36]), "+f"(d[37]), "+f"(d[38]), "+f"(d[39]), "+f"(d[40]), "+f"(d[41]), "+f"(d[42]), "+f"(d[43]), "+f"(d[44]), "+f"(d[45]), "+f"(d[46]), "+f"(d[47]), "+f"(d[48]), "+f"(d[49]), "+f"(d[50]), "+f"(d[51]), "+f"(d[52]), "+f"(d[53]), "+f"(d[54]), "+f"(d[55]), "+f"(d[56]), "+f"(d[57]), "+f"(d[58]), "+f"(d[59]), "+f"(d[60]), "+f"(d[61]), "+f"(d[62]), "+f"(d[63]), "+f"(d[64]), "+f"(d[65]), "+f"(d[66]), "+f"(d[67]), "+f"(d[68]), "+f"(d[69]), "+f"(d[70]), "+f"(d[71]), "+f"(d[72]), "+f"(d[73]), "+f"(d[74]), "+f"(d[75]), "+f"(d[76]), "+f"(d[77]), "+f"(d[78]), "+f"(d[79]), "+f"(d[80]), "+f"(d[81]), "+f"(d[82]), "+f"(d[83]), "+f"(d[84]), "+f"(d[85]), "+f"(d[86]), "+f"(d[87]), "+f"(d[88]), "+f"(d[89]), "+f"(d[90]), "+f"(d[91]), "+f"(d[92]), "+f"(d[93]), "+f"(d[94]), "+f"(d[95])
      : "l"(da), "l"(db), "r"(scale_d));
}
__device__ __forceinline__ void wgmma_ss_n256_bf16(float (&d)[128], uint64_t da, uint64_t db, uint32_t scale_d) {
  asm volatile(
      "{\n\t.reg .pred p;\n\t"
      "setp.ne.b32 p, %130, 0;\n\t"
      "wgmma.mma_async.sync.aligned.m64n256k16.f32.bf16.bf16 "
      "{%0, %1, %2, %3, %4, %5, %6, %7, %8, %9, %10, %11, %12, %13, %14, %15, %16, %17, %18, %19, %20, %21, %22, %23, %24, %25, %26, %27, %28, %29, %30, %31, %32, %33, %34, %35, %36, %37, %38, %39, %40, %41, %42, %43, %44, %45, %46, %47, %48, %49, %50, %51, %52, %53, %54, %55, %56, %57, %58, %59, %60, %61, %62, %63, %64, %65, %66, %67, %68, %69, %70, %71, %72, %73, %74, %75, %76, %77, %78, %79, %80, %81, %82, %83, %84, %85, %86, %87, %88, %89, %90, %91, %92, %93, %94, %95, %96, %97, %98, %99, %100, %101, %102, %103, %104, %105, %106, %107, %108, %109, %110, %111, %112, %113, %114, %115, %116, %117, %118, %119, %120, %121, %122, %123, %124, %125, %126, %127}, "
      "%128, %129, p, 1, 1, 0, 0;\n\t}"
      : "+f"(d[0]), "+f"(d[1]), "+f"(d[2]), "+f"(d[3]), "+f"(d[4]), "+f"(d[5]), "+f"(d[6]), "+f"(d[7]), "+f"(d[8]), "+f"(d[9]), "+f"(d[10]), "+f"(d[11]), "+f"(d[12]), "+f"(d[13]), "+f"(d[14]), "+f"(d[15]), "+f"(d[16]), "+f"(d[17]), "+f"(d[18]), "+f"(d[19]), "+f"(d[20]), "+f"(d[21]), "+f"(d[22]), "+f"(d[23]), "+f"(d[24]), "+f"(d[25]), "+f"(d[26]), "+f"(d[27]), "+f"(d[28]), "+f"(d[29]), "+f"(d[30]), "+f"(d[31]), "+f"(d[32]), "+f"(d[33]), "+f"(d[34]), "+f"(d[35]), "+f"(d[36]), "+f"(d[37]), "+f"(d[38]), "+f"(d[39]), "+f"(d[40]), "+f"(d[41]), "+f"(d[42]), "+f"(d[43]), "+f"(d[44]), "+f"(d[45]), "+f"(d[46]), "+f"(d[47]), "+f"(d[48]), "+f"(d[49]), "+f"(d[50]), "+f"(d[51]), "+f"(d[52]), "+f"(d[53]), "+f"(d[54]), "+f"(d[55]), "+f"(d[56]), "+f"(d[57]), "+f"(d[58]), "+f"(d[59]), "+f"(d[60]), "+f"(d[61]), "+f"(d[62]), "+f"(d[63]), "+f"(d[64]), "+f"(d[65]), "+f"(d[66]), "+f"(d[67]), "+f"(d[68]), "+f"(d[69]), "+f"(d[70]), "+f"(d[71]), "+f"(d[72]), "+f"(d[73]), "+f"(d[74]), "+f"(d[75]), "+f"(d[76]), "+f"(d[77]), "+f"(d[78]), "+f"(d[79]), "+f"(d[80]), "+f"(d[81]), "+f"(d[82]), "+f"(d[83]), "+f"(d[84]), "+f"(d[85]), "+f"(d[86]), "+f"(d[87]), "+f"(d[88]), "+f"(d[89]), "+f"(d[90]), "+f"(d[91]), "+f"(d[92]), "+f"(d[93]), "+f"(d[94]), "+f"(d[95]), "+f"(d[96]), "+f"(d[97]), "+f"(d[98]), "+f"(d[99]), "+f"(d[100]), "+f"(d[101]), "+f"(d[102]), "+f"(d[103]), "+f"(d[104]), "+f"(d[105]), "+f"(d[106]), "+f"(d[107]), "+f"(d[108]), "+f"(d[109]), "+f"(d[110]), "+f"(d[111]), "+f"(d[112]), "+f"(d[113]), "+f"(d[114]), "+f"(d[115]), "+f"(d[116]), "+f"(d[117]), "+f"(d[118]), "+f"(d[119]), "+f"(d[120]), "+f"(d[121]), "+f"(d[122]), "+f"(d[123]), "+f"(d[124]), "+f"(d[125]), "+f"(d[126]), "+f"(d[127])
      : "l"(da), "l"(db), "r"(scale_d));
}
__device__ __forceinline__ void wgmma_ss_n256_f16(float (&d)[128], uint64_t da, uint64_t db, uint32_t scale_d) {
  asm volatile(
      "{\n\t.reg .pred p;\n\t"
      "setp.ne.b32 p, %130, 0;\n\t"
      "wgmma.mma_async.sync.aligned.m64n256k16.f32.f16.f16 "
      "{%0, %1, %2, %3, %4, %5, %6, %7, %8, %9, %10, %11, %12, %13, %14, %15, %16, %17, %18, %19, %20, %21, %22, %23, %24, %25, %26, %27, %28, %29, %30, %31, %32, %33, %34, %35, %36, %37, %38, %39, %40, %41, %42, %43, %44, %45, %46, %47, %48, %49, %50, %51, %52, %53, %54, %55, %56, %57, %58, %59, %60, %61, %62, %63, %64, %65, %66, %67, %68, %69, %70, %71, %72, %73, %74, %75, %76, %77, %78, %79, %80, %81, %82, %83, %84, %85, %86, %87, %88, %89, %90, %91, %92, %93, %94, %95, %96, %97, %98, %99, %100, %101, %102, %103, %104, %105, %106, %107, %108, %109, %110, %111, %112, %113, %114, %115, %116, %117, %118, %119, %120, %121, %122, %123, %124, %125, %126, %127}, "
      "%128, %129, p, 1, 1, 0, 0;\n\t}"
      : "+f"(d[0]), "+f"(d[1]), "+f"(d[2]), "+f"(d[3]), "+f"(d[4]), "+f"(d[5]), "+f"(d[6]), "+f"(d[7]), "+f"(d[8]), "+f"(d[9]), "+f"(d[10]), "+f"(d[11]), "+f"(d[12]), "+f"(d[13]), "+f"(d[14]), "+f"(d[15]), "+f"(d[16]), "+f"(d[17]), "+f"(d[18]), "+f"(d[19]), "+f"(d[20]), "+f"(d[21]), "+f"(d[22]), "+f"(d[23]), "+f"(d[24]), "+f"(d[25]), "+f"(d[26]), "+f"(d[27]), "+f"(d[28]), "+f"(d[29]), "+f"(d[30]), "+f"(d[31]), "+f"(d[32]), "+f"(d[33]), "+f"(d[34]), "+f"(d[35]), "+f"(d[36]), "+f"(d[37]), "+f"(d[38]), "+f"(d[39]), "+f"(d[40]), "+f"(d[41]), "+f"(d[42]), "+f"(d[43]), "+f"(d[44]), "+f"(d[45]), "+f"(d[46]), "+f"(d[47]), "+f"(d[48]), "+f"(d[49]), "+f"(d[50]), "+f"(d[51]), "+f"(d[52]), "+f"(d[53]), "+f"(d[54]), "+f"(d[55]), "+f"(d[56]), "+f"(d[57]), "+f"(d[58]), "+f"(d[59]), "+f"(d[60]), "+f"(d[61]), "+f"(d[62]), "+f"(d[63]), "+f"(d[64]), "+f"(d[65]), "+f"(d[66]), "+f"(d[67]), "+f"(d[68]), "+f"(d[69]), "+f"(d[70]), "+f"(d[71]), "+f"(d[72]), "+f"(d[73]), "+f"(d[74]), "+f"(d[75]), "+f"(d[76]), "+f"(d[77]), "+f"(d[78]), "+f"(d[79]), "+f"(d[80]), "+f"(d[81]), "+f"(d[82]), "+f"(d[83]), "+f"(d[84]), "+f"(d[85]), "+f"(d[86]), "+f"(d[87]), "+f"(d[88]), "+f"(d[89]), "+f"(d[90]), "+f"(d[91]), "+f"(d[92]), "+f"(d[93]), "+f"(d[94]), "+f"(d[95]), "+f"(d[96]), "+f"(d[97]), "+f"(d[98]), "+f"(d[99]), "+f"(d[100]), "+f"(d[101]), "+f"(d[102]), "+f"(d[103]), "+f"(d[104]), "+f"(d[105]), "+f"(d[106]), "+f"(d[107]), "+f"(d[108]), "+f"(d[109]), "+f"(d[110]), "+f"(d[111]), "+f"(d[112]), "+f"(d[113]), "+f"(d[114]), "+f"(d[115]), "+f"(d[116]), "+f"(d[117]), "+f"(d[118]), "+f"(d[119]), "+f"(d[120]), "+f"(d[121]), "+f"(d[122]), "+f"(d[123]), "+f"(d[124]), "+f"(d[125]), "+f"(d[126]), "+f"(d[127])
      : "l"(da), "l"(db), "r"(scale_d));
}
__device__ __forceinline__ void wgmma_rs_n64_bf16_tb(float (&d)[32], const uint32_t (&a)[4], uint64_t db, uint32_t scale_d) {
  asm volatile(
      "{\n\t.reg .pred p;\n\t"
      "setp.ne.b32 p, %37, 0;\n\t"
      "wgmma.mma_async.sync.aligned.m64n64k16.f32.bf16.bf16 "
      "{%0, %1, %2, %3, %4, %5, %6, %7, %8, %9, %10, %11, %12, %13, %14, %15, %16, %17, %18, %19, %20, %21, %22, %23, %24, %25, %26, %27, %28, %29, %30, %31}, "
      "{%32, %33, %34, %35}, %36, p, 1, 1, 1;\n\t}"
      : "+f"(d[0]), "+f"(d[1]), "+f"(d[2]), "+f"(d[3]), "+f"(d[4]), "+f"(d[5]), "+f"(d[6]), "+f"(d[7]), "+f"(d[8]), "+f"(d[9]), "+f"(d[10]), "+f"(d[11]), "+f"(d[12]), "+f"(d[13]), "+f"(d[14]), "+f"(d[15]), "+f"(d[16]), "+f"(d[17]), "+f"(d[18]), "+f"(d[19]), "+f"(d[20]), "+f"(d[21]), "+f"(d[22]), "+f"(d[23]), "+f"(d[24]), "+f"(d[25]), "+f"(d[26]), "+f"(d[27]), "+f"(d[28]), "+f"(d[29]), "+f"(d[30]), "+f"(d[31])
      : "r"(a[0]), "r"(a[1]), "r"(a[2]), "r"(a[3]), "l"(db), "r"(scale_d));
}

__device__ __forceinline__ void wgmma_fence() { asm volatile("wgmma.fence.sync.aligned;" ::: "memory"); }
__device__ __forceinline__ void wgmma_commit() { asm volatile("wgmma.commit_group.sync.aligned;" ::: "memory"); }
template <int kPending>
__device__ __forceinline__ void wgmma_wait() { asm volatile("wgmma.wait_group.sync.aligned %0;" ::"n"(kPending) : "memory"); }
template <int kN>
__device__ __forceinline__ void acc_fence(float (&d)[kN]) {
#pragma unroll
  for (int i = 0; i < kN; ++i) asm volatile("" : "+f"(d[i])::"memory");
}

}
```

Before: 538.6.

## Split GEMM tile into two N-halves per consumer warpgroup with register reallocation

Restructures the shared ViT/conv GEMM so each consumer warpgroup owns one 128-column (or 96-column) half of the 256-wide tile. Each warpgroup computes both 64-row M halves with n128 wgmma instead of n256. The producer streams the two halves through a 5-stage ring with per-warpgroup full barriers, and setmaxnreg moves registers from the producer warps to the consumers. The epilogue stages through small per-warpgroup chunk buffers rather than reusing the operand ring, which lets the ring-free barrier go. The aim is to overlap one half's epilogue with the other half's MMA and deepen the pipeline. In exchange, the A operand is loaded twice per tile, and the smem and barrier layout becomes more complex.

```diff
diff --git a/gigapose_b200/csrc/api.cu b/gigapose_b200/csrc/api.cu
--- a/gigapose_b200/csrc/api.cu
+++ b/gigapose_b200/csrc/api.cu
@@ -334,9 +334,9 @@
         (e = gp_internal_make_map_raw(&h->tm_h1s_lo, h1_lo, 2, dims, strides, box, estr)) ||
         (e = gp_internal_make_map_raw(&h->tm_h1i_hi, h1_hi + 512, 2, dims, strides, box, estr)) ||
         (e = gp_internal_make_map_raw(&h->tm_h1i_lo, h1_lo + 512, 2, dims, strides, box, estr)) ||
-        (e = gp_internal_make_map(&h->tm_w1_hi, h->ws.w1_hi, 1024, 512, 256)) || (e = gp_internal_make_map(&h->tm_w1_lo, h->ws.w1_lo, 1024, 512, 256)) ||
-        (e = gp_internal_make_map(&h->tm_w2s_hi, h->ws.w2s_hi, 256, 512, 256)) || (e = gp_internal_make_map(&h->tm_w2s_lo, h->ws.w2s_lo, 256, 512, 256)) ||
-        (e = gp_internal_make_map(&h->tm_w2i_hi, h->ws.w2i_hi, 256, 512, 256)) || (e = gp_internal_make_map(&h->tm_w2i_lo, h->ws.w2i_lo, 256, 512, 256))) {
+        (e = gp_internal_make_map(&h->tm_w1_hi, h->ws.w1_hi, 1024, 512, 128)) || (e = gp_internal_make_map(&h->tm_w1_lo, h->ws.w1_lo, 1024, 512, 128)) ||
+        (e = gp_internal_make_map(&h->tm_w2s_hi, h->ws.w2s_hi, 256, 512, 128)) || (e = gp_internal_make_map(&h->tm_w2s_lo, h->ws.w2s_lo, 256, 512, 128)) ||
+        (e = gp_internal_make_map(&h->tm_w2i_hi, h->ws.w2i_hi, 256, 512, 128)) || (e = gp_internal_make_map(&h->tm_w2i_lo, h->ws.w2i_lo, 256, 512, 128))) {
       delete h;
       return e;
     }
diff --git a/gigapose_b200/csrc/ist_trunk.cu b/gigapose_b200/csrc/ist_trunk.cu
--- a/gigapose_b200/csrc/ist_trunk.cu
+++ b/gigapose_b200/csrc/ist_trunk.cu
@@ -246,7 +246,7 @@
       ce = gp::launch_split_planes(w[i].weight, c.cout, c.K, c.Kpad, c.w.hi, c.w.lo, s);
     }
     if (ce != cudaSuccess) break;
-    const uint32_t wbox = c.swap ? 128 : c.bn, pix_tile = c.swap ? 256 : 128;
+    const uint32_t wbox = c.swap ? 128 : c.bn / 2, pix_tile = 128;
     if ((e = gp_internal_make_map(&c.w_hi, c.w.hi, c.cout, c.Kpad, wbox)) || (e = gp_internal_make_map(&c.w_lo, c.w.lo, c.cout, c.Kpad, wbox)))
       break;
     if (c.in_buf < 0) {
diff --git a/gigapose_b200/csrc/vit_api.cu b/gigapose_b200/csrc/vit_api.cu
--- a/gigapose_b200/csrc/vit_api.cu
+++ b/gigapose_b200/csrc/vit_api.cu
@@ -124,7 +124,7 @@
 
   h->patch_b = w[1]; h->cls = w[2]; h->pos = w[3];
   cudaError_t ce = gp::launch_split_planes(w[0], kDim, kPatchK, kPatchKPad, h->patch_w.hi, h->patch_w.lo, s);
-  int e = ce == cudaSuccess ? make_maps(&h->patch_w, kDim, kPatchKPad, 256) : GP_ERR_CUDA;
+  int e = ce == cudaSuccess ? make_maps(&h->patch_w, kDim, kPatchKPad, 128) : GP_ERR_CUDA;
   for (int i = 0; i < depth && !e && ce == cudaSuccess; ++i) {
     const float* const* b = w + 4 + 14 * i;
     BlockW& B = h->blocks[i];
@@ -134,8 +134,8 @@
     if ((ce = gp::launch_split_planes(b[4], kDim, kDim, kDim, B.proj.hi, B.proj.lo, s)) != cudaSuccess) break;
     if ((ce = gp::launch_split_planes(b[9], kMlp, kDim, kDim, B.fc1.hi, B.fc1.lo, s)) != cudaSuccess) break;
     if ((ce = gp::launch_split_planes(b[11], kDim, kMlp, kMlp, B.fc2.hi, B.fc2.lo, s)) != cudaSuccess) break;
-    if ((e = make_maps(&B.qkv, kQkv, kDim, 256)) || (e = make_maps(&B.proj, kDim, kDim, 256)) ||
-        (e = make_maps(&B.fc1, kMlp, kDim, 256)) || (e = make_maps(&B.fc2, kDim, kMlp, 256)))
+    if ((e = make_maps(&B.qkv, kQkv, kDim, 128)) || (e = make_maps(&B.proj, kDim, kDim, 128)) ||
+        (e = make_maps(&B.fc1, kMlp, kDim, 128)) || (e = make_maps(&B.fc2, kDim, kMlp, 128)))
       break;
   }
   const uint64_t M = (uint64_t)max_crops * kTok;
@@ -197,8 +197,8 @@
   auto* w_h = const_cast<uint16_t*>(d->w_hi); auto* w_l = const_cast<uint16_t*>(d->w_lo);
   if (int e = gp_internal_make_map(&a_hi, a_h, g.M, g.K, 128)) return e;
   if (int e = gp_internal_make_map(&a_lo, a_l, g.M, g.K, 128)) return e;
-  if (int e = gp_internal_make_map(&w_hi, w_h, g.N, g.K, bn)) return e;
-  if (int e = gp_internal_make_map(&w_lo, w_l, g.N, g.K, bn)) return e;
+  if (int e = gp_internal_make_map(&w_hi, w_h, g.N, g.K, bn / 2)) return e;
+  if (int e = gp_internal_make_map(&w_lo, w_l, g.N, g.K, bn / 2)) return e;
   GPV_CUDA(gp::launch_vit_gemm(a_hi, a_lo, w_hi, w_lo, g, sms, static_cast<cudaStream_t>(stream)));
   gp_internal_count_launches(1);
   return GP_OK;
diff --git a/gigapose_b200/csrc/vit_gemm.cu b/gigapose_b200/csrc/vit_gemm.cu
--- a/gigapose_b200/csrc/vit_gemm.cu
+++ b/gigapose_b200/csrc/vit_gemm.cu
@@ -10,25 +10,30 @@
 
 constexpr int kBlockK = 32;
 constexpr int kRowBytes = kBlockK * 2;
-constexpr int kStages = 4;
 constexpr int kBM = 128, kBN = 256;
+constexpr int kHalfN = kBN / 2;
 constexpr int kAPlane = kBM * kRowBytes;
-constexpr int kWPlane = kBN * kRowBytes;
+constexpr int kWPlane = kHalfN * kRowBytes;
 constexpr int kStageBytes = 2 * kAPlane + 2 * kWPlane;
+constexpr int kStages = 5;
 constexpr int kEpiWarps = 8;
 constexpr int kThreads = 4 * 32 + kEpiWarps * 32;
-constexpr int kAccPitch = kBN + 4;
-static_assert(kBM * kAccPitch * 4 <= kStages * kStageBytes, "the staged accumulator lives in the operand ring");
+constexpr int kChunkCols = 32;
+constexpr int kChunkPitch = kChunkCols + 4;
+constexpr int kLaunchRegs = 168;
+constexpr int kProducerRegs = 40, kConsumerRegs = 232;
+static_assert(128 * kProducerRegs + 256 * kConsumerRegs <= kLaunchRegs * kThreads, "setmaxnreg exceeds the CTA's registers");
 
 struct __align__(8) GemmSmemTail {
-  float bias_s[2][kBN];
-  float gamma_s[2][kBN];
+  float chunk[2][kBM * kChunkPitch];
+  float bias_s[2][kHalfN];
+  float gamma_s[2][kHalfN];
   uint8_t stage_buf[kEpiWarps][32 * 80];
-  uint64_t full_bar[kStages];
+  uint64_t full_bar[2][kStages];
   uint64_t empty_bar[kStages];
-  uint64_t ring_free_bar;
 };
 constexpr int kSmemBytes = 1024 + kStages * kStageBytes + sizeof(GemmSmemTail);
+static_assert(kSmemBytes <= 227 * 1024, "shared memory");
 
 constexpr int kGroupM = 16;
 __device__ __forceinline__ void tile_coords(int tile, int num_m, int num_n, int& m_tile, int& n_tile) {
@@ -60,24 +65,60 @@
 }
 
 __device__ long long g_gemm_stamp[64];
-#define GSTAMP(i) do { if (blockIdx.x == 0 && p.N == 3072 && (i) < 64) g_gemm_stamp[i] = clock64(); } while (0)
-
-template <int kN, bool kF16>
-__device__ __forceinline__ void gemm_kblock(float (&d)[kN / 2], uint32_t a_hi, uint32_t a_lo, uint32_t w_hi, uint32_t w_lo,
-                                            int passes, bool first) {
-#pragma unroll
-  for (int pass = 0; pass < 3; ++pass) {
-    if (pass < passes) {
-      const uint32_t a = (pass == 2 ? a_lo : a_hi), w = (pass == 1 ? w_lo : w_hi);
-#pragma unroll
-      for (int k16 = 0; k16 < kBlockK / 16; ++k16) {
-        const uint64_t da = wgmma_desc_kmajor<kRowBytes>(a + k16 * 32), dw = wgmma_desc_kmajor<kRowBytes>(w + k16 * 32);
-        const uint32_t accum = (!first || pass != 0 || k16 != 0) ? 1u : 0u;
-        if constexpr (kN == 256) { if constexpr (kF16) wgmma_ss_n256_f16(d, da, dw, accum); else wgmma_ss_n256_bf16(d, da, dw, accum); }
-        if constexpr (kN == 192) { if constexpr (kF16) wgmma_ss_n192_f16(d, da, dw, accum); else wgmma_ss_n192_bf16(d, da, dw, accum); }
+#define GSTAMP(i) do { if (blockIdx.x == 0 && p.N == 3072) g_gemm_stamp[i] = clock64(); } while (0)
+
+namespace {
+
+template <int kRegs> __device__ __forceinline__ void setmaxnreg_dec() { asm volatile("setmaxnreg.dec.sync.aligned.u32 %0;" ::"n"(kRegs)); }
+template <int kRegs> __device__ __forceinline__ void setmaxnreg_inc() { asm volatile("setmaxnreg.inc.sync.aligned.u32 %0;" ::"n"(kRegs)); }
+
+template <int kPasses, int kN, bool kF16>
+__device__ __forceinline__ void gemm_kblock(float (&d0)[kN / 2], float (&d1)[kN / 2], uint32_t a_hi, uint32_t a_lo,
+                                            uint32_t w_hi, uint32_t w_lo, bool first) {
+#pragma unroll
+  for (int pass = 0; pass < kPasses; ++pass) {
+    const uint32_t a = (pass == 2 ? a_lo : a_hi), w = (pass == 1 ? w_lo : w_hi);
+#pragma unroll
+    for (int k16 = 0; k16 < kBlockK / 16; ++k16) {
+      const uint64_t da0 = wgmma_desc_kmajor<kRowBytes>(a + k16 * 32);
+      const uint64_t da1 = wgmma_desc_kmajor<kRowBytes>(a + kAPlane / 2 + k16 * 32);
+      const uint64_t dw = wgmma_desc_kmajor<kRowBytes>(w + k16 * 32);
+      const uint32_t accum = (!first || pass != 0 || k16 != 0) ? 1u : 0u;
+      if constexpr (kN == 128) {
+        if constexpr (kF16) { wgmma_ss_n128_f16(d0, da0, dw, accum); wgmma_ss_n128_f16(d1, da1, dw, accum); }
+        else { wgmma_ss_n128_bf16(d0, da0, dw, accum); wgmma_ss_n128_bf16(d1, da1, dw, accum); }
+      } else {
+        static_assert(kN == 96 && !kF16, "column halves: 128 (bf16, fp16) or 96 (bf16)");
+        wgmma_ss_n96_bf16(d0, da0, dw, accum); wgmma_ss_n96_bf16(d1, da1, dw, accum);
       }
     }
   }
+}
+
+template <int kPasses, int kN, bool kF16>
+__device__ __forceinline__ void gemm_unit_mma(float (&d0)[kN / 2], float (&d1)[kN / 2], uint8_t* smem, GemmSmemTail& tail,
+                                              int wg, int num_kb, int& slot, uint32_t& phases, int lane) {
+  int prev = -1;
+  for (int kb = 0; kb < num_kb; ++kb) {
+    mbar_wait(&tail.full_bar[wg][slot], (phases >> slot) & 1u);
+    phases ^= 1u << slot;
+    const uint32_t st = smem_u32(smem + slot * kStageBytes);
+    acc_fence(d0);
+    acc_fence(d1);
+    wgmma_fence();
+    gemm_kblock<kPasses, kN, kF16>(d0, d1, st, st + kAPlane, st + 2 * kAPlane, st + 2 * kAPlane + kWPlane, kb == 0);
+    wgmma_commit();
+    wgmma_wait<1>();
+    if (prev >= 0 && lane == 0) mbar_arrive(&tail.empty_bar[prev]);
+    prev = slot;
+    if (++slot == kStages) slot = 0;
+  }
+  wgmma_wait<0>();
+  acc_fence(d0);
+  acc_fence(d1);
+  if (lane == 0) mbar_arrive(&tail.empty_bar[prev]);
+}
+
 }
 
 template <bool kSwap, int kTileN, bool kF16, int kMode>
@@ -88,18 +129,21 @@
   pdl_trigger();
   uint8_t* smem = smem_raw + ((1024u - (smem_u32(smem_raw) & 1023u)) & 1023u);
   GemmSmemTail& tail = *reinterpret_cast<GemmSmemTail*>(smem + kStages * kStageBytes);
-  float* acc_s = reinterpret_cast<float*>(smem);
   const int warp = threadIdx.x >> 5, lane = threadIdx.x & 31;
   const int passes = p.passes;
-  constexpr int bn = kTileN;
-  const int M_rows = p.m_dev ? min(*p.m_dev, p.M) : p.M;
-  const int num_m = (M_rows + kBM - 1) / kBM, num_n = p.N / bn;
-  const int num_tiles = num_m * num_n;
-  const int num_kb = p.K / kBlockK;
+  constexpr int bn = kTileN, half_cols = bn / 2;
+#define GEMM_TILE_COUNTS                                                                                            \
+  const int M_rows = p.m_dev ? min(*p.m_dev, p.M) : p.M;  \
+  const int num_m = (M_rows + kBM - 1) / kBM, num_n = p.N / bn;                                                    \
+  const int num_tiles = num_m * num_n;                                                                             \
+  const int num_kb = p.K / kBlockK
 
   if (threadIdx.x == 0) {
-    for (int s = 0; s < kStages; ++s) { mbar_init(&tail.full_bar[s], 1); mbar_init(&tail.empty_bar[s], kEpiWarps); }
-    mbar_init(&tail.ring_free_bar, kEpiWarps);
+    for (int s = 0; s < kStages; ++s) {
+      mbar_init(&tail.full_bar[0][s], 1);
+      mbar_init(&tail.full_bar[1][s], 1);
+      mbar_init(&tail.empty_bar[s], 4);
+    }
     fence_barrier_init();
   }
   if (warp == 0 && lane == 0) {
@@ -108,107 +152,79 @@
   }
   __syncthreads();
   pdl_wait();
-  if (threadIdx.x == 0) GSTAMP(63);
-
-  if (warp == 0) {
-    if (lane == 0) {
-      int stage = 0; uint32_t phase = 0, unit = 0;
-      const uint32_t tx = (passes == 3 ? 2 : 1) * (kAPlane + bn * kRowBytes);
-      for (int tile = blockIdx.x; tile < num_tiles; tile += gridDim.x, ++unit) {
+  if (threadIdx.x == 0) { GSTAMP(63); if (blockIdx.x == 0 && p.N == 3072) g_gemm_stamp[62] = 2; }
+
+  if (warp < 4) {
+    setmaxnreg_dec<kProducerRegs>();
+    if (warp == 0 && lane == 0) {
+      GEMM_TILE_COUNTS;
+      int stage = 0; uint32_t phase = 0;
+      const uint32_t tx = (passes == 3 ? 2 : 1) * (kAPlane + half_cols * kRowBytes);
+      for (int tile = blockIdx.x; tile < num_tiles; tile += gridDim.x) {
         int mt, nt;
         tile_coords(tile, num_m, num_n, mt, nt);
-        const int m0 = mt * kBM, n0 = nt * bn;
-        int img = 0, y0 = 0;
-        if (p.conv) { const int hw = p.Ho * p.Wo, pix0 = kSwap ? n0 : m0; img = pix0 / hw; y0 = (pix0 - img * hw) / p.Wo; }
-        if (unit > 0) mbar_wait(&tail.ring_free_bar, (unit - 1) & 1u);
-        for (int kb = 0; kb < num_kb; ++kb) {
-          mbar_wait(&tail.empty_bar[stage], phase ^ 1);
-          uint8_t* st = smem + stage * kStageBytes;
-          mbar_arrive_expect_tx(&tail.full_bar[stage], tx);
-          int cb = 0, cx = 0, cy = 0;
-          if (p.conv) {
-            const int tap = kb / p.cblocks;
-            cb = kb - tap * p.cblocks;
-            const int ky = tap / p.kw, kx = tap - ky * p.kw;
-            cx = kx - p.pad; cy = y0 * p.stride + ky - p.pad;
-          }
-          auto load2 = [&](void* dst, const CUtensorMap* map, int c0, int c1) { tma_load_2d(dst, map, &tail.full_bar[stage], c0, c1); };
-          auto load4 = [&](void* dst, const CUtensorMap* map) {
-            tma_load_4d(dst, map, &tail.full_bar[stage], cb * kBlockK, cx, cy, img);
-          };
-          if (p.conv && !kSwap) {
-            load4(st, &tm_a_hi);
-            if (passes == 3) load4(st + kAPlane, &tm_a_lo);
-          } else {
-            load2(st, &tm_a_hi, kb * kBlockK, m0);
-            if (passes == 3) load2(st + kAPlane, &tm_a_lo, kb * kBlockK, m0);
-          }
-          if (p.conv && kSwap) {
-            load4(st + 2 * kAPlane, &tm_w_hi);
-            if (passes == 3) load4(st + 2 * kAPlane + kWPlane, &tm_w_lo);
-          } else {
-            load2(st + 2 * kAPlane, &tm_w_hi, kb * kBlockK, n0);
-            if (passes == 3) load2(st + 2 * kAPlane + kWPlane, &tm_w_lo, kb * kBlockK, n0);
-          }
-          if (++stage == kStages) { stage = 0; phase ^= 1; }
+        const int m0 = mt * kBM;
+        for (int h = 0; h < 2; ++h) {
+          const int n0 = nt * bn + h * half_cols;
+          uint64_t* full = tail.full_bar[h];
+          int img = 0, y0 = 0;
+          if (p.conv) { const int hw = p.Ho * p.Wo, pix0 = kSwap ? n0 : m0; img = pix0 / hw; y0 = (pix0 - img * hw) / p.Wo; }
+          for (int kb = 0; kb < num_kb; ++kb) {
+            mbar_wait(&tail.empty_bar[stage], phase ^ 1);
+            uint8_t* st = smem + stage * kStageBytes;
+            mbar_arrive_expect_tx(&full[stage], tx);
+            int cb = 0, cx = 0, cy = 0;
+            if (p.conv) {
+              const int tap = kb / p.cblocks;
+              cb = kb - tap * p.cblocks;
+              const int ky = tap / p.kw, kx = tap - ky * p.kw;
+              cx = kx - p.pad; cy = y0 * p.stride + ky - p.pad;
+            }
+            auto load2 = [&](void* dst, const CUtensorMap* map, int c0, int c1) { tma_load_2d(dst, map, &full[stage], c0, c1); };
+            auto load4 = [&](void* dst, const CUtensorMap* map) { tma_load_4d(dst, map, &full[stage], cb * kBlockK, cx, cy, img); };
+            if (p.conv && !kSwap) {
+              load4(st, &tm_a_hi);
+              if (passes == 3) load4(st + kAPlane, &tm_a_lo);
+            } else {
+              load2(st, &tm_a_hi, kb * kBlockK, m0);
+              if (passes == 3) load2(st + kAPlane, &tm_a_lo, kb * kBlockK, m0);
+            }
+            if (p.conv && kSwap) {
+              load4(st + 2 * kAPlane, &tm_w_hi);
+              if (passes == 3) load4(st + 2 * kAPlane + kWPlane, &tm_w_lo);
+            } else {
+              load2(st + 2 * kAPlane, &tm_w_hi, kb * kBlockK, n0);
+              if (passes == 3) load2(st + 2 * kAPlane + kWPlane, &tm_w_lo, kb * kBlockK, n0);
+            }
+            if (++stage == kStages) { stage = 0; phase ^= 1; }
+          }
         }
       }
     }
-  } else if (warp >= 4) {
-    const int e = warp - 4, q = e & 3, ch = e >> 2;
+  } else {
+    setmaxnreg_inc<kConsumerRegs>();
+    GEMM_TILE_COUNTS;
+    const int e = warp - 4, q = e & 3, wg = e >> 2;
     const int r = q * 32 + lane;
-    const int etid = e * 32 + lane;
-    const int wg = e >> 2, wl = e & 3;
-    int stage = 0; uint32_t phase = 0, unit = 0;
+    const uint32_t bar_id = 1 + wg;
+    float* chunk = tail.chunk[wg];
+    int slot = (wg * num_kb) % kStages;
+    uint32_t phases = 0;
+    int unit = 0;
     for (int tile = blockIdx.x; tile < num_tiles; tile += gridDim.x, ++unit) {
-      const uint32_t acc_i = unit & 1u;
       int mt, nt;
       tile_coords(tile, num_m, num_n, mt, nt);
-      if (e == 0 && lane == 0) GSTAMP(unit * 4 + 0);
-      float frag[kTileN / 2];
-      int prev_stage = -1;
-      for (int kb = 0; kb < num_kb; ++kb) {
-        mbar_wait(&tail.full_bar[stage], phase);
-        const uint32_t st = smem_u32(smem + stage * kStageBytes);
-        const uint32_t a_hi = st + wg * (kAPlane / 2), a_lo = a_hi + kAPlane;
-        const uint32_t w_hi = st + 2 * kAPlane, w_lo = w_hi + kWPlane;
-        acc_fence(frag);
-        wgmma_fence();
-        gemm_kblock<kTileN, kF16>(frag, a_hi, a_lo, w_hi, w_lo, passes, kb == 0);
-        wgmma_commit();
-        wgmma_wait<1>();
-        if (prev_stage >= 0 && lane == 0) mbar_arrive(&tail.empty_bar[prev_stage]);
-        prev_stage = stage;
-        if (++stage == kStages) { stage = 0; phase ^= 1; }
-      }
-      wgmma_wait<0>();
-      acc_fence(frag);
-      if (lane == 0) mbar_arrive(&tail.empty_bar[prev_stage]);
-      if (e == 0 && lane == 0) GSTAMP(unit * 4 + 1);
-      named_barrier_sync(1, kEpiWarps * 32);
-      {
-        const int row0 = wg * 64 + wl * 16 + (lane >> 2), col0 = 2 * (lane & 3);
-#pragma unroll
-        for (int j8 = 0; j8 < kTileN / 8; ++j8) {
-          {
-            *reinterpret_cast<float2*>(acc_s + row0 * kAccPitch + j8 * 8 + col0) = make_float2(frag[4 * j8], frag[4 * j8 + 1]);
-            *reinterpret_cast<float2*>(acc_s + (row0 + 8) * kAccPitch + j8 * 8 + col0) = make_float2(frag[4 * j8 + 2], frag[4 * j8 + 3]);
-          }
-        }
-      }
-      const int ntile0 = nt * bn;
-      if (!kSwap && etid < bn) {
-        tail.bias_s[acc_i][etid] = __ldg(p.bias + ntile0 + etid);
-        if (kMode == GEMM_SCALE_RESIDUAL) tail.gamma_s[acc_i][etid] = __ldg(p.gamma + ntile0 + etid);
-      }
-      named_barrier_sync(1, kEpiWarps * 32);
-      if (e == 0 && lane == 0) GSTAMP(unit * 4 + 2);
-      const uint32_t acc = acc_i;
+      const bool stamp = q == 0 && lane == 0 && unit < 7;
+      if (stamp) GSTAMP(32 * wg + 4 * unit + 0);
+      float acc0[half_cols / 2], acc1[half_cols / 2];
+      if (passes == 3) gemm_unit_mma<3, half_cols, kF16>(acc0, acc1, smem, tail, wg, num_kb, slot, phases, lane);
+      else gemm_unit_mma<1, half_cols, kF16>(acc0, acc1, smem, tail, wg, num_kb, slot, phases, lane);
+      slot = (slot + num_kb) % kStages;
+      if (stamp) GSTAMP(32 * wg + 4 * unit + 1);
       const int m = mt * kBM + r;
-      const int half_cols = bn >> 1;
-      const int n0 = ntile0 + ch * half_cols;
-      const float* sb = tail.bias_s[acc] + ch * half_cols;
-      const float* sg = tail.gamma_s[acc] + ch * half_cols;
+      const int n0 = nt * bn + wg * half_cols;
+      const float* sb = tail.bias_s[wg];
+      const float* sg = tail.gamma_s[wg];
       const bool row_ok = m < M_rows;
       size_t out_row = (size_t)m;
       const float* pos_row = nullptr;
@@ -377,22 +393,43 @@
         }
       };
 
-      const float* arow = acc_s + r * kAccPitch + ch * half_cols;
-      for (int c0 = 0; c0 < half_cols; c0 += 32) {
+      if (stamp) GSTAMP(32 * wg + 4 * unit + 2);
+      constexpr int kChunks = half_cols / kChunkCols;
+      const int row0 = q * 16 + (lane >> 2), col0 = 2 * (lane & 3);
+      for (int c = 0; c < kChunks; ++c) {
+        named_barrier_sync(bar_id, 128);
+#pragma unroll
+        for (int cc = 0; cc < kChunks; ++cc) {
+          if (cc == c) {
+#pragma unroll
+            for (int jj = 0; jj < kChunkCols / 8; ++jj) {
+              const int j8 = cc * (kChunkCols / 8) + jj;
+              float* dst = chunk + row0 * kChunkPitch + jj * 8 + col0;
+              *reinterpret_cast<float2*>(dst) = make_float2(acc0[4 * j8], acc0[4 * j8 + 1]);
+              *reinterpret_cast<float2*>(dst + 8 * kChunkPitch) = make_float2(acc0[4 * j8 + 2], acc0[4 * j8 + 3]);
+              *reinterpret_cast<float2*>(dst + 64 * kChunkPitch) = make_float2(acc1[4 * j8], acc1[4 * j8 + 1]);
+              *reinterpret_cast<float2*>(dst + 72 * kChunkPitch) = make_float2(acc1[4 * j8 + 2], acc1[4 * j8 + 3]);
+            }
+          }
+        }
+        if (!kSwap && c == 0 && r < half_cols) {
+          tail.bias_s[wg][r] = __ldg(p.bias + n0 + r);
+          if (kMode == GEMM_SCALE_RESIDUAL) tail.gamma_s[wg][r] = __ldg(p.gamma + n0 + r);
+        }
+        named_barrier_sync(bar_id, 128);
+        const float* arow = chunk + r * kChunkPitch;
         uint32_t v[32];
 #pragma unroll
         for (int j = 0; j < 8; ++j) {
-          const uint4 t = *reinterpret_cast<const uint4*>(arow + c0 + 4 * j);
+          const uint4 t = *reinterpret_cast<const uint4*>(arow + 4 * j);
           v[4 * j] = t.x; v[4 * j + 1] = t.y; v[4 * j + 2] = t.z; v[4 * j + 3] = t.w;
         }
-        process(v, c0);
+        process(v, c * kChunkCols);
       }
-      fence_proxy_async();
-      __syncwarp();
-      if (lane == 0) mbar_arrive(&tail.ring_free_bar);
-      if (e == 0 && lane == 0) GSTAMP(unit * 4 + 3);
+      if (stamp) GSTAMP(32 * wg + 4 * unit + 3);
     }
   }
+#undef GEMM_TILE_COUNTS
 }
 
 cudaError_t read_gemm_stamps(long long* host64) { return cudaMemcpyFromSymbol(host64, g_gemm_stamp, sizeof(long long) * 64); }
@@ -406,6 +443,9 @@
   if (!configured) {
     cudaError_t e = cudaFuncSetAttribute(kernel, cudaFuncAttributeMaxDynamicSharedMemorySize, kSmemBytes);
     if (e != cudaSuccess) return e;
+    cudaFuncAttributes fa;
+    if ((e = cudaFuncGetAttributes(&fa, kernel)) != cudaSuccess) return e;
+    if (fa.numRegs != kLaunchRegs) return cudaErrorInvalidKernelImage;
     configured = true;
   }
   return launch_ex(kernel, dim3(grid), dim3(kThreads), kSmemBytes, stream, 1, true, a_hi, a_lo, w_hi, w_lo, p);
@@ -422,8 +462,8 @@
   if (p.K <= 0 || p.K % kBlockK != 0) return no("K must be a positive multiple of 32");
   if (p.passes != 1 && p.passes != 3) return no("passes must be 1 or 3");
   if (p.mode < GEMM_PLANES || p.mode > GEMM_ROWS_F32_RELU) return no("unknown mode");
-  const int tile_pixels = p.swap ? bn : kBM;
-  if (p.conv && (p.Wo <= 0 || tile_pixels % p.Wo != 0 || p.M % kBM != 0 || p.cblocks <= 0))
+  const int box_pixels = p.swap ? bn / 2 : kBM;
+  if (p.conv && (p.Wo <= 0 || box_pixels % p.Wo != 0 || p.M % kBM != 0 || p.cblocks <= 0))
     return no("convolution geometry does not tile");
   if (p.swap && (bn != kBN || p.M % kBM != 0 || p.f16 || !plane_mode))
     return no("swap needs bn = 256, M % 128 == 0, bf16 planes and a plane mode without GELU");
diff --git a/gigapose_b200/csrc/wgmma.cuh b/gigapose_b200/csrc/wgmma.cuh
--- a/gigapose_b200/csrc/wgmma.cuh
+++ b/gigapose_b200/csrc/wgmma.cuh
@@ -43,24 +43,34 @@
       : "+f"(d[0]), "+f"(d[1]), "+f"(d[2]), "+f"(d[3]), "+f"(d[4]), "+f"(d[5]), "+f"(d[6]), "+f"(d[7]), "+f"(d[8]), "+f"(d[9]), "+f"(d[10]), "+f"(d[11]), "+f"(d[12]), "+f"(d[13]), "+f"(d[14]), "+f"(d[15]), "+f"(d[16]), "+f"(d[17]), "+f"(d[18]), "+f"(d[19]), "+f"(d[20]), "+f"(d[21]), "+f"(d[22]), "+f"(d[23]), "+f"(d[24]), "+f"(d[25]), "+f"(d[26]), "+f"(d[27]), "+f"(d[28]), "+f"(d[29]), "+f"(d[30]), "+f"(d[31])
       : "l"(da), "l"(db), "r"(scale_d));
 }
-__device__ __forceinline__ void wgmma_ss_n192_bf16(float (&d)[96], uint64_t da, uint64_t db, uint32_t scale_d) {
+__device__ __forceinline__ void wgmma_ss_n96_bf16(float (&d)[48], uint64_t da, uint64_t db, uint32_t scale_d) {
   asm volatile(
       "{\n\t.reg .pred p;\n\t"
-      "setp.ne.b32 p, %98, 0;\n\t"
-      "wgmma.mma_async.sync.aligned.m64n192k16.f32.bf16.bf16 "
-      "{%0, %1, %2, %3, %4, %5, %6, %7, %8, %9, %10, %11, %12, %13, %14, %15, %16, %17, %18, %19, %20, %21, %22, %23, %24, %25, %26, %27, %28, %29, %30, %31, %32, %33, %34, %35, %36, %37, %38, %39, %40, %41, %42, %43, %44, %45, %46, %47, %48, %49, %50, %51, %52, %53, %54, %55, %56, %57, %58, %59, %60, %61, %62, %63, %64, %65, %66, %67, %68, %69, %70, %71, %72, %73, %74, %75, %76, %77, %78, %79, %80, %81, %82, %83, %84, %85, %86, %87, %88, %89, %90, %91, %92, %93, %94, %95}, "
-      "%96, %97, p, 1, 1, 0, 0;\n\t}"
-      : "+f"(d[0]), "+f"(d[1]), "+f"(d[2]), "+f"(d[3]), "+f"(d[4]), "+f"(d[5]), "+f"(d[6]), "+f"(d[7]), "+f"(d[8]), "+f"(d[9]), "+f"(d[10]), "+f"(d[11]), "+f"(d[12]), "+f"(d[13]), "+f"(d[14]), "+f"(d[15]), "+f"(d[16]), "+f"(d[17]), "+f"(d[18]), "+f"(d[19]), "+f"(d[20]), "+f"(d[21]), "+f"(d[22]), "+f"(d[23]), "+f"(d[24]), "+f"(d[25]), "+f"(d[26]), "+f"(d[27]), "+f"(d[28]), "+f"(d[29]), "+f"(d[30]), "+f"(d[31]), "+f"(d[32]), "+f"(d[33]), "+f"(d[34]), "+f"(d[35]), "+f"(d[36]), "+f"(d[37]), "+f"(d[38]), "+f"(d[39]), "+f"(d[40]), "+f"(d[41]), "+f"(d[42]), "+f"(d[43]), "+f"(d[44]), "+f"(d[45]), "+f"(d[46]), "+f"(d[47]), "+f"(d[48]), "+f"(d[49]), "+f"(d[50]), "+f"(d[51]), "+f"(d[52]), "+f"(d[53]), "+f"(d[54]), "+f"(d[55]), "+f"(d[56]), "+f"(d[57]), "+f"(d[58]), "+f"(d[59]), "+f"(d[60]), "+f"(d[61]), "+f"(d[62]), "+f"(d[63]), "+f"(d[64]), "+f"(d[65]), "+f"(d[66]), "+f"(d[67]), "+f"(d[68]), "+f"(d[69]), "+f"(d[70]), "+f"(d[71]), "+f"(d[72]), "+f"(d[73]), "+f"(d[74]), "+f"(d[75]), "+f"(d[76]), "+f"(d[77]), "+f"(d[78]), "+f"(d[79]), "+f"(d[80]), "+f"(d[81]), "+f"(d[82]), "+f"(d[83]), "+f"(d[84]), "+f"(d[85]), "+f"(d[86]), "+f"(d[87]), "+f"(d[88]), "+f"(d[89]), "+f"(d[90]), "+f"(d[91]), "+f"(d[92]), "+f"(d[93]), "+f"(d[94]), "+f"(d[95])
+      "setp.ne.b32 p, %50, 0;\n\t"
+      "wgmma.mma_async.sync.aligned.m64n96k16.f32.bf16.bf16 "
+      "{%0, %1, %2, %3, %4, %5, %6, %7, %8, %9, %10, %11, %12, %13, %14, %15, %16, %17, %18, %19, %20, %21, %22, %23, %24, %25, %26, %27, %28, %29, %30, %31, %32, %33, %34, %35, %36, %37, %38, %39, %40, %41, %42, %43, %44, %45, %46, %47}, "
+      "%48, %49, p, 1, 1, 0, 0;\n\t}"
+      : "+f"(d[0]), "+f"(d[1]), "+f"(d[2]), "+f"(d[3]), "+f"(d[4]), "+f"(d[5]), "+f"(d[6]), "+f"(d[7]), "+f"(d[8]), "+f"(d[9]), "+f"(d[10]), "+f"(d[11]), "+f"(d[12]), "+f"(d[13]), "+f"(d[14]), "+f"(d[15]), "+f"(d[16]), "+f"(d[17]), "+f"(d[18]), "+f"(d[19]), "+f"(d[20]), "+f"(d[21]), "+f"(d[22]), "+f"(d[23]), "+f"(d[24]), "+f"(d[25]), "+f"(d[26]), "+f"(d[27]), "+f"(d[28]), "+f"(d[29]), "+f"(d[30]), "+f"(d[31]), "+f"(d[32]), "+f"(d[33]), "+f"(d[34]), "+f"(d[35]), "+f"(d[36]), "+f"(d[37]), "+f"(d[38]), "+f"(d[39]), "+f"(d[40]), "+f"(d[41]), "+f"(d[42]), "+f"(d[43]), "+f"(d[44]), "+f"(d[45]), "+f"(d[46]), "+f"(d[47])
       : "l"(da), "l"(db), "r"(scale_d));
 }
-__device__ __forceinline__ void wgmma_ss_n192_f16(float (&d)[96], uint64_t da, uint64_t db, uint32_t scale_d) {
+__device__ __forceinline__ void wgmma_ss_n128_bf16(float (&d)[64], uint64_t da, uint64_t db, uint32_t scale_d) {
   asm volatile(
       "{\n\t.reg .pred p;\n\t"
-      "setp.ne.b32 p, %98, 0;\n\t"
-      "wgmma.mma_async.sync.aligned.m64n192k16.f32.f16.f16 "
-      "{%0, %1, %2, %3, %4, %5, %6, %7, %8, %9, %10, %11, %12, %13, %14, %15, %16, %17, %18, %19, %20, %21, %22, %23, %24, %25, %26, %27, %28, %29, %30, %31, %32, %33, %34, %35, %36, %37, %38, %39, %40, %41, %42, %43, %44, %45, %46, %47, %48, %49, %50, %51, %52, %53, %54, %55, %56, %57, %58, %59, %60, %61, %62, %63, %64, %65, %66, %67, %68, %69, %70, %71, %72, %73, %74, %75, %76, %77, %78, %79, %80, %81, %82, %83, %84, %85, %86, %87, %88, %89, %90, %91, %92, %93, %94, %95}, "
-      "%96, %97, p, 1, 1, 0, 0;\n\t}"
-      : "+f"(d[0]), "+f"(d[1]), "+f"(d[2]), "+f"(d[3]), "+f"(d[4]), "+f"(d[5]), "+f"(d[6]), "+f"(d[7]), "+f"(d[8]), "+f"(d[9]), "+f"(d[10]), "+f"(d[11]), "+f"(d[12]), "+f"(d[13]), "+f"(d[14]), "+f"(d[15]), "+f"(d[16]), "+f"(d[17]), "+f"(d[18]), "+f"(d[19]), "+f"(d[20]), "+f"(d[21]), "+f"(d[22]), "+f"(d[23]), "+f"(d[24]), "+f"(d[25]), "+f"(d[26]), "+f"(d[27]), "+f"(d[28]), "+f"(d[29]), "+f"(d[30]), "+f"(d[31]), "+f"(d[32]), "+f"(d[33]), "+f"(d[34]), "+f"(d[35]), "+f"(d[36]), "+f"(d[37]), "+f"(d[38]), "+f"(d[39]), "+f"(d[40]), "+f"(d[41]), "+f"(d[42]), "+f"(d[43]), "+f"(d[44]), "+f"(d[45]), "+f"(d[46]), "+f"(d[47]), "+f"(d[48]), "+f"(d[49]), "+f"(d[50]), "+f"(d[51]), "+f"(d[52]), "+f"(d[53]), "+f"(d[54]), "+f"(d[55]), "+f"(d[56]), "+f"(d[57]), "+f"(d[58]), "+f"(d[59]), "+f"(d[60]), "+f"(d[61]), "+f"(d[62]), "+f"(d[63]), "+f"(d[64]), "+f"(d[65]), "+f"(d[66]), "+f"(d[67]), "+f"(d[68]), "+f"(d[69]), "+f"(d[70]), "+f"(d[71]), "+f"(d[72]), "+f"(d[73]), "+f"(d[74]), "+f"(d[75]), "+f"(d[76]), "+f"(d[77]), "+f"(d[78]), "+f"(d[79]), "+f"(d[80]), "+f"(d[81]), "+f"(d[82]), "+f"(d[83]), "+f"(d[84]), "+f"(d[85]), "+f"(d[86]), "+f"(d[87]), "+f"(d[88]), "+f"(d[89]), "+f"(d[90]), "+f"(d[91]), "+f"(d[92]), "+f"(d[93]), "+f"(d[94]), "+f"(d[95])
+      "setp.ne.b32 p, %66, 0;\n\t"
+      "wgmma.mma_async.sync.aligned.m64n128k16.f32.bf16.bf16 "
+      "{%0, %1, %2, %3, %4, %5, %6, %7, %8, %9, %10, %11, %12, %13, %14, %15, %16, %17, %18, %19, %20, %21, %22, %23, %24, %25, %26, %27, %28, %29, %30, %31, %32, %33, %34, %35, %36, %37, %38, %39, %40, %41, %42, %43, %44, %45, %46, %47, %48, %49, %50, %51, %52, %53, %54, %55, %56, %57, %58, %59, %60, %61, %62, %63}, "
+      "%64, %65, p, 1, 1, 0, 0;\n\t}"
+      : "+f"(d[0]), "+f"(d[1]), "+f"(d[2]), "+f"(d[3]), "+f"(d[4]), "+f"(d[5]), "+f"(d[6]), "+f"(d[7]), "+f"(d[8]), "+f"(d[9]), "+f"(d[10]), "+f"(d[11]), "+f"(d[12]), "+f"(d[13]), "+f"(d[14]), "+f"(d[15]), "+f"(d[16]), "+f"(d[17]), "+f"(d[18]), "+f"(d[19]), "+f"(d[20]), "+f"(d[21]), "+f"(d[22]), "+f"(d[23]), "+f"(d[24]), "+f"(d[25]), "+f"(d[26]), "+f"(d[27]), "+f"(d[28]), "+f"(d[29]), "+f"(d[30]), "+f"(d[31]), "+f"(d[32]), "+f"(d[33]), "+f"(d[34]), "+f"(d[35]), "+f"(d[36]), "+f"(d[37]), "+f"(d[38]), "+f"(d[39]), "+f"(d[40]), "+f"(d[41]), "+f"(d[42]), "+f"(d[43]), "+f"(d[44]), "+f"(d[45]), "+f"(d[46]), "+f"(d[47]), "+f"(d[48]), "+f"(d[49]), "+f"(d[50]), "+f"(d[51]), "+f"(d[52]), "+f"(d[53]), "+f"(d[54]), "+f"(d[55]), "+f"(d[56]), "+f"(d[57]), "+f"(d[58]), "+f"(d[59]), "+f"(d[60]), "+f"(d[61]), "+f"(d[62]), "+f"(d[63])
+      : "l"(da), "l"(db), "r"(scale_d));
+}
+__device__ __forceinline__ void wgmma_ss_n128_f16(float (&d)[64], uint64_t da, uint64_t db, uint32_t scale_d) {
+  asm volatile(
+      "{\n\t.reg .pred p;\n\t"
+      "setp.ne.b32 p, %66, 0;\n\t"
+      "wgmma.mma_async.sync.aligned.m64n128k16.f32.f16.f16 "
+      "{%0, %1, %2, %3, %4, %5, %6, %7, %8, %9, %10, %11, %12, %13, %14, %15, %16, %17, %18, %19, %20, %21, %22, %23, %24, %25, %26, %27, %28, %29, %30, %31, %32, %33, %34, %35, %36, %37, %38, %39, %40, %41, %42, %43, %44, %45, %46, %47, %48, %49, %50, %51, %52, %53, %54, %55, %56, %57, %58, %59, %60, %61, %62, %63}, "
+      "%64, %65, p, 1, 1, 0, 0;\n\t}"
+      : "+f"(d[0]), "+f"(d[1]), "+f"(d[2]), "+f"(d[3]), "+f"(d[4]), "+f"(d[5]), "+f"(d[6]), "+f"(d[7]), "+f"(d[8]), "+f"(d[9]), "+f"(d[10]), "+f"(d[11]), "+f"(d[12]), "+f"(d[13]), "+f"(d[14]), "+f"(d[15]), "+f"(d[16]), "+f"(d[17]), "+f"(d[18]), "+f"(d[19]), "+f"(d[20]), "+f"(d[21]), "+f"(d[22]), "+f"(d[23]), "+f"(d[24]), "+f"(d[25]), "+f"(d[26]), "+f"(d[27]), "+f"(d[28]), "+f"(d[29]), "+f"(d[30]), "+f"(d[31]), "+f"(d[32]), "+f"(d[33]), "+f"(d[34]), "+f"(d[35]), "+f"(d[36]), "+f"(d[37]), "+f"(d[38]), "+f"(d[39]), "+f"(d[40]), "+f"(d[41]), "+f"(d[42]), "+f"(d[43]), "+f"(d[44]), "+f"(d[45]), "+f"(d[46]), "+f"(d[47]), "+f"(d[48]), "+f"(d[49]), "+f"(d[50]), "+f"(d[51]), "+f"(d[52]), "+f"(d[53]), "+f"(d[54]), "+f"(d[55]), "+f"(d[56]), "+f"(d[57]), "+f"(d[58]), "+f"(d[59]), "+f"(d[60]), "+f"(d[61]), "+f"(d[62]), "+f"(d[63])
       : "l"(da), "l"(db), "r"(scale_d));
 }
 __device__ __forceinline__ void wgmma_ss_n256_bf16(float (&d)[128], uint64_t da, uint64_t db, uint32_t scale_d) {
@@ -68,16 +78,6 @@
       "{\n\t.reg .pred p;\n\t"
       "setp.ne.b32 p, %130, 0;\n\t"
       "wgmma.mma_async.sync.aligned.m64n256k16.f32.bf16.bf16 "
-      "{%0, %1, %2, %3, %4, %5, %6, %7, %8, %9, %10, %11, %12, %13, %14, %15, %16, %17, %18, %19, %20, %21, %22, %23, %24, %25, %26, %27, %28, %29, %30, %31, %32, %33, %34, %35, %36, %37, %38, %39, %40, %41, %42, %43, %44, %45, %46, %47, %48, %49, %50, %51, %52, %53, %54, %55, %56, %57, %58, %59, %60, %61, %62, %63, %64, %65, %66, %67, %68, %69, %70, %71, %72, %73, %74, %75, %76, %77, %78, %79, %80, %81, %82, %83, %84, %85, %86, %87, %88, %89, %90, %91, %92, %93, %94, %95, %96, %97, %98, %99, %100, %101, %102, %103, %104, %105, %106, %107, %108, %109, %110, %111, %112, %113, %114, %115, %116, %117, %118, %119, %120, %121, %122, %123, %124, %125, %126, %127}, "
-      "%128, %129, p, 1, 1, 0, 0;\n\t}"
-      : "+f"(d[0]), "+f"(d[1]), "+f"(d[2]), "+f"(d[3]), "+f"(d[4]), "+f"(d[5]), "+f"(d[6]), "+f"(d[7]), "+f"(d[8]), "+f"(d[9]), "+f"(d[10]), "+f"(d[11]), "+f"(d[12]), "+f"(d[13]), "+f"(d[14]), "+f"(d[15]), "+f"(d[16]), "+f"(d[17]), "+f"(d[18]), "+f"(d[19]), "+f"(d[20]), "+f"(d[21]), "+f"(d[22]), "+f"(d[23]), "+f"(d[24]), "+f"(d[25]), "+f"(d[26]), "+f"(d[27]), "+f"(d[28]), "+f"(d[29]), "+f"(d[30]), "+f"(d[31]), "+f"(d[32]), "+f"(d[33]), "+f"(d[34]), "+f"(d[35]), "+f"(d[36]), "+f"(d[37]), "+f"(d[38]), "+f"(d[39]), "+f"(d[40]), "+f"(d[41]), "+f"(d[42]), "+f"(d[43]), "+f"(d[44]), "+f"(d[45]), "+f"(d[46]), "+f"(d[47]), "+f"(d[48]), "+f"(d[49]), "+f"(d[50]), "+f"(d[51]), "+f"(d[52]), "+f"(d[53]), "+f"(d[54]), "+f"(d[55]), "+f"(d[56]), "+f"(d[57]), "+f"(d[58]), "+f"(d[59]), "+f"(d[60]), "+f"(d[61]), "+f"(d[62]), "+f"(d[63]), "+f"(d[64]), "+f"(d[65]), "+f"(d[66]), "+f"(d[67]), "+f"(d[68]), "+f"(d[69]), "+f"(d[70]), "+f"(d[71]), "+f"(d[72]), "+f"(d[73]), "+f"(d[74]), "+f"(d[75]), "+f"(d[76]), "+f"(d[77]), "+f"(d[78]), "+f"(d[79]), "+f"(d[80]), "+f"(d[81]), "+f"(d[82]), "+f"(d[83]), "+f"(d[84]), "+f"(d[85]), "+f"(d[86]), "+f"(d[87]), "+f"(d[88]), "+f"(d[89]), "+f"(d[90]), "+f"(d[91]), "+f"(d[92]), "+f"(d[93]), "+f"(d[94]), "+f"(d[95]), "+f"(d[96]), "+f"(d[97]), "+f"(d[98]), "+f"(d[99]), "+f"(d[100]), "+f"(d[101]), "+f"(d[102]), "+f"(d[103]), "+f"(d[104]), "+f"(d[105]), "+f"(d[106]), "+f"(d[107]), "+f"(d[108]), "+f"(d[109]), "+f"(d[110]), "+f"(d[111]), "+f"(d[112]), "+f"(d[113]), "+f"(d[114]), "+f"(d[115]), "+f"(d[116]), "+f"(d[117]), "+f"(d[118]), "+f"(d[119]), "+f"(d[120]), "+f"(d[121]), "+f"(d[122]), "+f"(d[123]), "+f"(d[124]), "+f"(d[125]), "+f"(d[126]), "+f"(d[127])
-      : "l"(da), "l"(db), "r"(scale_d));
-}
-__device__ __forceinline__ void wgmma_ss_n256_f16(float (&d)[128], uint64_t da, uint64_t db, uint32_t scale_d) {
-  asm volatile(
-      "{\n\t.reg .pred p;\n\t"
-      "setp.ne.b32 p, %130, 0;\n\t"
-      "wgmma.mma_async.sync.aligned.m64n256k16.f32.f16.f16 "
       "{%0, %1, %2, %3, %4, %5, %6, %7, %8, %9, %10, %11, %12, %13, %14, %15, %16, %17, %18, %19, %20, %21, %22, %23, %24, %25, %26, %27, %28, %29, %30, %31, %32, %33, %34, %35, %36, %37, %38, %39, %40, %41, %42, %43, %44, %45, %46, %47, %48, %49, %50, %51, %52, %53, %54, %55, %56, %57, %58, %59, %60, %61, %62, %63, %64, %65, %66, %67, %68, %69, %70, %71, %72, %73, %74, %75, %76, %77, %78, %79, %80, %81, %82, %83, %84, %85, %86, %87, %88, %89, %90, %91, %92, %93, %94, %95, %96, %97, %98, %99, %100, %101, %102, %103, %104, %105, %106, %107, %108, %109, %110, %111, %112, %113, %114, %115, %116, %117, %118, %119, %120, %121, %122, %123, %124, %125, %126, %127}, "
       "%128, %129, p, 1, 1, 0, 0;\n\t}"
       : "+f"(d[0]), "+f"(d[1]), "+f"(d[2]), "+f"(d[3]), "+f"(d[4]), "+f"(d[5]), "+f"(d[6]), "+f"(d[7]), "+f"(d[8]), "+f"(d[9]), "+f"(d[10]), "+f"(d[11]), "+f"(d[12]), "+f"(d[13]), "+f"(d[14]), "+f"(d[15]), "+f"(d[16]), "+f"(d[17]), "+f"(d[18]), "+f"(d[19]), "+f"(d[20]), "+f"(d[21]), "+f"(d[22]), "+f"(d[23]), "+f"(d[24]), "+f"(d[25]), "+f"(d[26]), "+f"(d[27]), "+f"(d[28]), "+f"(d[29]), "+f"(d[30]), "+f"(d[31]), "+f"(d[32]), "+f"(d[33]), "+f"(d[34]), "+f"(d[35]), "+f"(d[36]), "+f"(d[37]), "+f"(d[38]), "+f"(d[39]), "+f"(d[40]), "+f"(d[41]), "+f"(d[42]), "+f"(d[43]), "+f"(d[44]), "+f"(d[45]), "+f"(d[46]), "+f"(d[47]), "+f"(d[48]), "+f"(d[49]), "+f"(d[50]), "+f"(d[51]), "+f"(d[52]), "+f"(d[53]), "+f"(d[54]), "+f"(d[55]), "+f"(d[56]), "+f"(d[57]), "+f"(d[58]), "+f"(d[59]), "+f"(d[60]), "+f"(d[61]), "+f"(d[62]), "+f"(d[63]), "+f"(d[64]), "+f"(d[65]), "+f"(d[66]), "+f"(d[67]), "+f"(d[68]), "+f"(d[69]), "+f"(d[70]), "+f"(d[71]), "+f"(d[72]), "+f"(d[73]), "+f"(d[74]), "+f"(d[75]), "+f"(d[76]), "+f"(d[77]), "+f"(d[78]), "+f"(d[79]), "+f"(d[80]), "+f"(d[81]), "+f"(d[82]), "+f"(d[83]), "+f"(d[84]), "+f"(d[85]), "+f"(d[86]), "+f"(d[87]), "+f"(d[88]), "+f"(d[89]), "+f"(d[90]), "+f"(d[91]), "+f"(d[92]), "+f"(d[93]), "+f"(d[94]), "+f"(d[95]), "+f"(d[96]), "+f"(d[97]), "+f"(d[98]), "+f"(d[99]), "+f"(d[100]), "+f"(d[101]), "+f"(d[102]), "+f"(d[103]), "+f"(d[104]), "+f"(d[105]), "+f"(d[106]), "+f"(d[107]), "+f"(d[108]), "+f"(d[109]), "+f"(d[110]), "+f"(d[111]), "+f"(d[112]), "+f"(d[113]), "+f"(d[114]), "+f"(d[115]), "+f"(d[116]), "+f"(d[117]), "+f"(d[118]), "+f"(d[119]), "+f"(d[120]), "+f"(d[121]), "+f"(d[122]), "+f"(d[123]), "+f"(d[124]), "+f"(d[125]), "+f"(d[126]), "+f"(d[127])
```

Measured after the change: 523.4, median of 6. 0.972x the previous value.
